# amoretti86/phylo

Measured on AMD Instinct MI355X. Metric: particle-site-likelihoods/sec, higher is better.
Workload: dtype f64; 1 GPU; primate.p N=12 S=898, GTR-init (jcmodel=false), K=2048 per GPU (K_total=2048), lambda=10, full sweep of 11 rank events; parallelism=particles sharded over 1 GPU(s), global resampling, sweeps_per_launch_set=16, contexts_in_flight=3, sweeps_in_flight=48, particles_in_flight=98304

## Files before the change

include/phylo_hip.h:

```cpp
#ifndef PHYLO_HIP_H
#define PHYLO_HIP_H

#include <stdint.h>

#ifdef __cplusplus
extern "C" {
#endif

typedef struct phylo_ctx phylo_ctx;

enum {
    PHYLO_OK = 0,
    PHYLO_EINVAL = -1,
    PHYLO_ENODEVICE = -2,
    PHYLO_EHIP = -3,
    PHYLO_ENOMEM = -4,
    PHYLO_ECOMM = -5,
    PHYLO_ESTATE = -6
};

enum {
    PHYLO_QUIRK_Q1_RAW_Q = 1u << 0,
    PHYLO_TWISTING = 1u << 1,
    PHYLO_TIME_KERNELS = 1u << 2,
// ... 98 lines not shown
                       phylo_stats* fwd, phylo_stats* bwd);
int phylo_vi_gradients_batch(phylo_ctx* ctx, const uint64_t* seeds, int G, uint32_t flags, int jc, const double* vars, double* logZ,
                             double* grads, phylo_stats* fwd, phylo_stats* bwd);
int phylo_vi_apply(int n_taxa, int jc, double* vars, const double* grads, int kind, double lr, double beta1, double beta2, double eps,
                   int64_t* t, double* m, double* v);

int phylo_debug_stamps(phylo_ctx* ctx, uint64_t* out, int n);

int phylo_debug_reverse_lists(int N, int K, const int64_t* ancestors, const int32_t* child, int early_free, int rows_form,
                              const int32_t* lookahead_nodes, int n_lookahead, int32_t* lists, int64_t n_lists, int32_t* meta,
                              int n_meta);

int phylo_debug_lookahead_lists(int N, int K, int S, int M, const int32_t* roots_ad, int32_t* slow_flag, int32_t* image,
                                int64_t n_image, int32_t* meta, int n_meta);

int phylo_debug_reverse_plan(int N, int K, int K_local, int S, int world, int twisted, int marks, uint32_t switches, int64_t n_slow,
                             int TS, int64_t coeff_wgs, int passes_in_flight, uint32_t* mask);
int phylo_debug_sweep_plan(int N, int K, int K_local, int S, int G, int M, int world, int transport, uint32_t flags, uint32_t switches,
                           uint32_t* mask, int32_t* launches);
int phylo_debug_sweep_chain(int N, int K, int K_local, int S, int G, int M, int world, int transport, uint32_t flags, uint32_t switches,
                            int multi_min, int scan_ancestors, int32_t* out);
int phylo_debug_sweep_chain_of(phylo_ctx* ctx, int32_t* taken);
int phylo_debug_scan_ancestors(phylo_ctx* ctx, const double* logw, int Kg, int G, const uint64_t* seeds, uint32_t r_next, int32_t* anc,
                               int32_t* list, int32_t* cnt);
int phylo_debug_scan_form(phylo_ctx* ctx, int Kg, int multi_min, int wanted);
int phylo_debug_persist_plan(int N, int K, int S, int G, uint32_t flags, uint32_t switches, int world, int transport, int n_cus,
                             int blocks_per_cu, int persist_wgs, int persist_nt, int64_t* out);
int phylo_debug_persist_of(phylo_ctx* ctx, int32_t* nt, int32_t* Wg, int32_t* m, int64_t* lds);
int phylo_debug_pack_leaf_codes(const uint8_t* codes, int N, int S, uint8_t* packed, int64_t cap, int64_t* need);
int phylo_debug_site_patterns(const uint8_t* codes, int N, int S, int32_t* U, int32_t* rep, uint16_t* image, uint32_t* rep_off,
                              uint8_t* rep_leaf, int64_t rep_leaf_cap);
int phylo_debug_site_patterns_rule(int S, int U, int coded, int ntiles, int sw);
int phylo_debug_site_patterns_of(phylo_ctx* ctx, int32_t* U, int32_t* taken);
int phylo_debug_reverse_plan_batch(int N, int K, int G, int S, uint32_t switches, int64_t n_slow, int TS, int64_t coeff_wgs,
                                   int passes_in_flight, uint32_t* mask);
int phylo_debug_tree_plan(int N, int K, int G, int world, int64_t n_clades, int64_t n_topologies, int kept_whole, int force_wide,
                          int64_t summary_temp, int64_t branches_temp, int64_t* scalars, int64_t* summary_slab, int64_t* branches_slab,
                          int32_t* sort_bits, int32_t* launches);
int phylo_debug_tree_branches_of(phylo_ctx* ctx, int32_t* wide, int32_t* cbits, int32_t* tbits);

int phylo_debug_device_lists(phylo_ctx* ctx, int32_t* lists, int64_t n_lists, int32_t* meta, int n_meta, int64_t* ancestors,
                             int32_t* child);
int phylo_debug_device_lists_of(phylo_ctx* ctx, const int64_t* ancestors, const int32_t* child, int32_t* lists, int64_t n_lists,
                                int32_t* meta, int n_meta);

int phylo_tree_summary(phylo_ctx* ctx, int64_t* n_clades, int32_t* n_topologies, int32_t* n_groups, phylo_stats* perf);
int phylo_tree_summary_fetch(phylo_ctx* ctx, uint64_t* clade_bits, uint64_t* clade_weight, int32_t* clade_group, uint64_t* topo_weight,
                             int32_t* topo_count, int32_t* topo_rep, int32_t* topo_group, int32_t* particle_topo, uint64_t* u, uint64_t* U);

int phylo_tree_branches(phylo_ctx* ctx, phylo_stats* perf);
int phylo_tree_branches_fetch(phylo_ctx* ctx, double* clade_stats, double* leaf_stats, int32_t* topo_clades, double* topo_stats);

int phylo_rell(phylo_ctx* ctx, int T, int S, const double* site_lik_TxS, int B, uint64_t seed, double* obs_T, int32_t* best_B,
               int64_t* wins_T, double* rep_loglik_TxB, int32_t* counts_BxS, double* site_loglik_TxS, phylo_stats* perf);
int phylo_debug_rell_host(int T, int S, const double* site_lik_TxS, int b0, int nB, uint64_t seed, int32_t* counts, double* x,
                          double* rl);
int phylo_rell_multiscale(phylo_ctx* ctx, int T, int S, const double* site_lik_TxS, int K, const int32_t* draws_K, int B, uint64_t seed,
                          double* obs_T, int64_t* wins_KxT, int32_t* best_KxB, double* rep_loglik_KxTxB, int32_t* counts_KxBxS,
                          phylo_stats* perf);
int phylo_debug_rell_multiscale_host(int T, int S, const double* site_lik_TxS, int K, const int32_t* draws_K, int k0, int b0, int nB,
                                     uint64_t seed, int32_t* counts, double* rl, int32_t* best);

int phylo_math_probe(phylo_ctx* ctx, int op, const double* x, const double* y, int n, double* out);

int phylo_debug_frechet(phylo_ctx* ctx, int form, const double* A_nx16, const double* E_nx16, int n, double* L_nx16);

// ... 18 lines not shown
```

phylo_amd/_ffi.py:

```python
from __future__ import annotations

import ctypes as C
import os

import numpy as np

_HERE = os.path.dirname(os.path.abspath(__file__))
LIB_PATH = os.path.join(_HERE, "csrc", "libphylo_hip.so")

PHYLO_OK = 0
QUIRK_Q1_RAW_Q = 1 << 0
TWISTING = 1 << 1
TIME_KERNELS = 1 << 2
EAGER_NODES = 1 << 3
KEEP_GRAPH = 1 << 4
ONE_LAUNCH = 1 << 5
FLAGS_DEFAULT = QUIRK_Q1_RAW_Q
COMM_ID_BYTES = 128

EXPORTS = [
    "phylo_version", "phylo_last_error", "phylo_device_count", "phylo_create", "phylo_destroy",
    "phylo_set_leaves", "phylo_set_model", "phylo_expm_batched", "phylo_cond_likelihood_K",
    "phylo_forest_loglik", "phylo_tree_loglik", "phylo_trees_loglik", "phylo_trees_loglik_rates", "phylo_trees_grad", "phylo_trees_grad_rates", "phylo_trees_grad_model", "phylo_trees_nni", "phylo_trees_nni_rates", "phylo_rell", "phylo_debug_rell_host", "phylo_rell_multiscale", "phylo_debug_rell_multiscale_host", "phylo_debug_tree_schedule", "phylo_resample", "phylo_log_zsmc", "phylo_sweep",
    "phylo_sweep_async", "phylo_sweep_batch_async", "phylo_sweep_batch_begin", "phylo_sweep_fetch_logz", "phylo_sweep_begin", "phylo_sweep_step", "phylo_sweep_step_a", "phylo_sweep_step_group", "phylo_sweep_finish", "phylo_sweep_fetch",
    "phylo_synchronize", "phylo_sweep_node", "phylo_sweep_backward", "phylo_sweep_backward_batch",
    "phylo_tree_summary", "phylo_tree_summary_fetch", "phylo_tree_branches", "phylo_tree_branches_fetch",
    "phylo_math_probe", "phylo_debug_frechet", "phylo_debug_stamps", "phylo_debug_reverse_lists", "phylo_debug_lookahead_lists", "phylo_debug_reverse_plan", "phylo_debug_reverse_plan_batch", "phylo_debug_sweep_plan", "phylo_debug_sweep_chain", "phylo_debug_sweep_chain_of", "phylo_debug_scan_ancestors", "phylo_debug_pack_leaf_codes", "phylo_debug_site_patterns", "phylo_debug_site_patterns_rule", "phylo_debug_site_patterns_of", "phylo_debug_tree_plan", "phylo_debug_tree_branches_of", "phylo_debug_scan_form", "phylo_debug_persist_plan", "phylo_debug_persist_of", "phylo_debug_device_lists", "phylo_debug_device_lists_of", "phylo_debug_remote_cache", "phylo_debug_site_product",
    "phylo_vi_gradients", "phylo_vi_gradients_batch", "phylo_vi_apply",
    "phylo_site_tile", "phylo_set_site_tile", "phylo_get_site_tile",
    "phylo_comm_unique_id", "phylo_comm_init", "phylo_comm_share", "phylo_comm_allgather", "phylo_comm_max", "phylo_comm_barrier",
    "phylo_comm_exchange_kind",
]


class PhyloError(RuntimeError):
    def __init__(self, code, msg):
        super().__init__("libphylo_hip error %d: %s" % (code, msg))
        self.code = code


class Stats(C.Structure):
    _fields_ = [("sweep_ms", C.c_double), ("merge_ms", C.c_double), ("merge_launches", C.c_int32),
                ("n_launches", C.c_int32), ("units", C.c_double), ("alg_bytes", C.c_double)]


_lib = None


def load():
    global _lib
    if _lib is None:
        if not os.path.exists(LIB_PATH):
            raise OSError("%s not found: build it with phylo_amd/csrc/build.sh (needs hipcc); "
                          "there is no CPU fallback" % LIB_PATH)
        lib = C.CDLL(LIB_PATH)
        lib.phylo_version.restype = C.c_char_p
        lib.phylo_last_error.restype = C.c_char_p
        lib.phylo_last_error.argtypes = [C.c_void_p]
        _lib = lib
    return _lib
# ... 125 lines not shown


SITE_PATTERN_SWITCH = {"0": 0, None: 1, "force": 2}


def debug_site_patterns(codes):
    lib = load()
    cd = np.ascontiguousarray(codes, dtype=np.uint8)
    if cd.ndim != 2:
        raise ValueError("codes must be [N][S]")
    N, S = cd.shape
    nC = -(-(-(-S // 64)) // 16)
    U = C.c_int32(0)
    rep = np.full(S, -1, dtype=np.int32)
    image = np.full(nC * 1024, 0xffff, dtype=np.uint16)
    rep_off = np.full(1024, 0xffffffff, dtype=np.uint32)
    rep_leaf = np.full(N * 1024, 0xff, dtype=np.uint8)
    rc = lib.phylo_debug_site_patterns(_ptr(cd), C.c_int(N), C.c_int(S), C.byref(U), _ptr(rep), _ptr(image), _ptr(rep_off), _ptr(rep_leaf),
                                       C.c_int64(rep_leaf.size))
    if rc:
        raise PhyloError(rc, lib.phylo_last_error(None).decode())
    u = U.value
    return {"U": u, "rep": rep[:u].copy(), "image": image.reshape(nC, 2, 64, 8) if u <= 8191 else None,
            "rep_off": rep_off if u <= 512 else None,
            "rep_leaf": rep_leaf[:N * 1024 * (-(-(-(-u // 64)) // 16))].reshape(N, -1, 64, 16) if u <= 512 else None}


def debug_site_patterns_rule(S, U, coded=True, ntiles=1, switch=None):
    lib = load()
    rc = lib.phylo_debug_site_patterns_rule(C.c_int(S), C.c_int(U), C.c_int(int(coded)), C.c_int(ntiles), C.c_int(SITE_PATTERN_SWITCH[switch]))
    if rc < 0:
        raise PhyloError(rc, lib.phylo_last_error(None).decode())
    return bool(rc)


TREE_SUMMARY_BUFS = ("u", "U", "bits", "kA", "kB", "val", "scan", "weight", "srt", "hp", "o_cbits", "o_cw", "o_tw", "child", "slot", "o_cg",
                     "o_tn", "o_trep", "o_tg", "o_ptopo", "vA", "vB", "flag", "sid", "cid", "seg_start", "count", "group", "first", "tid", "pos",
                     "err", "vC", "vD", "temp")
TREE_BRANCHES_BUFS = ("ebr", "lbr", "gbl", "gbr", "o_cs", "o_ls", "o_ts", "wA", "wB", "cpos", "kA", "kB", "vA", "vB", "cstart", "toff", "o_tc",
                      "temp")


def debug_tree_plan(N, K, G=1, world=1, n_clades=1, n_topologies=1, kept_whole=False, summary_temp=0, branches_temp=0, force_wide=False):
    lib = load()
    ns, nb = len(TREE_SUMMARY_BUFS), len(TREE_BRANCHES_BUFS)
    sc = (C.c_int64 * 13)()
    ss, bs = (C.c_int64 * (2 * ns + 1))(), (C.c_int64 * (2 * nb + 1))()
    bits, launches = (C.c_int32 * 17)(), (C.c_int32 * 2)()
    rc = lib.phylo_debug_tree_plan(C.c_int(N), C.c_int(K), C.c_int(G), C.c_int(world), C.c_int64(n_clades), C.c_int64(n_topologies),
                                   C.c_int(int(kept_whole)), C.c_int(int(force_wide)), C.c_int64(summary_temp), C.c_int64(branches_temp),
                                   sc, ss, bs, bits, launches)
    if rc:
        raise PhyloError(rc, lib.phylo_last_error(None).decode())
    out = dict(zip(("R", "L", "W", "E", "Emax", "Kg", "cbits", "tbits"), sc[:8]))
    out["wide"], out["gather"] = bool(sc[8]), bool(sc[9])
    if (sc[11], sc[12]) != (ns, nb):
        raise RuntimeError("TREE_SUMMARY_BUFS / TREE_BRANCHES_BUFS do not name the library's buffers")
    for key, names, a in (("summary_slab", TREE_SUMMARY_BUFS, ss), ("branches_slab", TREE_BRANCHES_BUFS, bs)):
        n = len(names)
        out[key] = {"offsets": dict(zip(names, a[:n])), "sizes": dict(zip(names, a[n:2 * n])), "total": a[2 * n]}
    out["sort_bits"] = list(bits[:sc[10]])
    out["summary_launches"], out["branches_launches"] = launches[0], launches[1]
    return out


SCAN_FORMS = ("multi", "lds512", "lds1024", "in_place")
# ... 648 lines not shown
        self._owner = owner
        world = owner.K // owner.K_local
        self.K_local = self.K // world
        self.k0 = (owner.k0 // owner.K_local) * self.K_local

    def comm_allgather_columns(self, a):
        a = np.ascontiguousarray(a)
        world = self.K // self.K_local
        if world == 1:
            return a
        out = np.empty((world,) + a.shape, dtype=a.dtype)
        self._check(self._lib.phylo_comm_allgather(self._h, _ptr(a), C.c_size_t(a.nbytes), _ptr(out)))
        return np.concatenate(list(out), axis=-1)

    def comm_allgather_blob(self, a):
        a = np.ascontiguousarray(a)
        world = self.K // self.K_local
        if world == 1:
            return a[None]
        out = np.empty((world,) + a.shape, dtype=a.dtype)
        self._check(self._lib.phylo_comm_allgather(self._h, _ptr(a), C.c_size_t(a.nbytes), _ptr(out)))
        return out

    def debug_remote_cache(self):
        used, cap = C.c_int(0), C.c_int(0)
        self._check(self._lib.phylo_debug_remote_cache(self._h, C.byref(used), C.byref(cap)))
        return used.value, cap.value

    def debug_site_patterns(self):
        U, taken = C.c_int32(0), C.c_int32(0)
        self._check(self._lib.phylo_debug_site_patterns_of(self._h, C.byref(U), C.byref(taken)))
        return U.value, bool(taken.value)

    def debug_tree_branches(self):
        wide, cbits, tbits = C.c_int32(0), C.c_int32(0), C.c_int32(0)
        self._check(self._lib.phylo_debug_tree_branches_of(self._h, C.byref(wide), C.byref(cbits), C.byref(tbits)))
        return {'wide': bool(wide.value), 'cbits': cbits.value, 'tbits': tbits.value}

    def debug_scan_form(self, Kg, wanted=True):
        rc = self._lib.phylo_debug_scan_form(self._h, C.c_int(Kg), C.c_int(0), C.c_int(int(wanted)))
        if rc < 0:
            raise PhyloError(rc, self._lib.phylo_last_error(self._h).decode())
        return SCAN_FORMS[rc]

    def debug_sweep_chain(self):
        taken = C.c_int32(0)
        self._check(self._lib.phylo_debug_sweep_chain_of(self._h, C.byref(taken)))
        return bool(taken.value)

    def debug_scan_ancestors(self, logw, seeds, r_next):
        w = np.ascontiguousarray(logw, dtype=np.float64)
        if w.ndim != 2:
            raise ValueError("logw must be [G][Kg]")
        G, Kg = w.shape
        sd = np.ascontiguousarray(seeds, dtype=np.uint64)
        if sd.shape != (G,):
            raise ValueError("one seed per group")
        anc = np.full((G, Kg), -2, dtype=np.int32)
        lst = np.full((G, Kg), -2, dtype=np.int32)
        cnt = np.full(G, -2, dtype=np.int32)
        self._check(self._lib.phylo_debug_scan_ancestors(self._h, _ptr(w), C.c_int(Kg), C.c_int(G), _ptr(sd), C.c_uint32(r_next), _ptr(anc),
                                                         _ptr(lst), _ptr(cnt)))
        return anc, lst, cnt

    def debug_persist(self):
        nt, Wg, m, lds = C.c_int32(0), C.c_int32(0), C.c_int32(0), C.c_int64(0)
# ... 29 lines not shown
```

phylo_amd/csrc/phylo_hip.hip:

```cpp
#include "../../include/phylo_hip.h"

#include <cstring>
#include <hip/hip_runtime.h>
#include <hip/hip_ext.h>
#include <rocprim/device/device_radix_sort.hpp>

#include <cstdarg>
#include <cstdio>
#include <cstdlib>
#include <atomic>
#include <chrono>
#include <mutex>
#include <string>
#include <vector>

#include "phylo_comm.h"
#include "phylo_kernels.h"
#include "phylo_packed_codes.h"
#include "phylo_site_patterns.h"
#include "phylo_persist.h"
#include "phylo_grad.h"
#include "phylo_revlists_dev.h"
#include "phylo_sweep_plan.h"
#include "phylo_train.h"
// ... 14 lines not shown
namespace {

thread_local std::string g_last_error;

struct DevBuf {
    void* p = nullptr;
    size_t bytes = 0;
};

}

struct sweep_run {
    uint64_t seed = 0;
    uint32_t flags = 0;
    int M = 1, launches = 0, next_r = 0;
    bool active = false;
    int a_done_r = -1;
    sweep_plan plan{};
    sweep_chain_form chain{};
};

struct env_switches {
    bool eager_nodes = false, rehearse_sharded = false, replicated_book = false, no_leaf_codes = false, one_launch = false,
         persist_stamps = false, grad_one_stream = false, grad_two_streams = false, rev_host_lists = false, no_remote_cache = false,
         no_p2p = false, grad_rows_chain = false, grad_coeff_chain = false, tree_wide_keys = false;
    int persist_wgs = 0;
    unsigned long long p2p_wait_ticks = PK_P2P_WAIT_TICKS;
    size_t p2p_copy_words = 65536;
    int persist_nt = 256;
    int remote_cache_cap = 0;
    int scan_multi_min = 4096;
    int scan_ancestors = 1;
    int site_patterns = PK_PAT_AUTO;
    int trees_chunk = 0;
    int rell_chunk = 0;
    void read() {
        eager_nodes = getenv("PHYLO_EAGER_NODES") != nullptr;
        rehearse_sharded = getenv("PHYLO_REHEARSE_SHARDED") != nullptr;
        replicated_book = getenv("PHYLO_REPLICATED_BOOK") != nullptr;
        grad_rows_chain = getenv("PHYLO_GRAD_ROWS_CHAIN") != nullptr;
        grad_coeff_chain = getenv("PHYLO_GRAD_COEFF_CHAIN") != nullptr;
        no_leaf_codes = getenv("PHYLO_NO_LEAF_CODES") != nullptr;
        one_launch = getenv("PHYLO_ONE_LAUNCH") != nullptr;
        persist_stamps = getenv("PHYLO_PERSIST_STAMPS") != nullptr;
        grad_one_stream = getenv("PHYLO_GRAD_ONE_STREAM") != nullptr;
        grad_two_streams = getenv("PHYLO_GRAD_TWO_STREAMS") != nullptr;
        rev_host_lists = getenv("PHYLO_REV_HOST_LISTS") != nullptr;
        no_remote_cache = getenv("PHYLO_NO_REMOTE_CACHE") != nullptr;
        { const char* e = getenv("PHYLO_TREE_WIDE_KEYS"); tree_wide_keys = e && atoi(e) != 0; }
        { const char* e = getenv("PHYLO_REMOTE_CACHE_CAP"); remote_cache_cap = e ? atoi(e) : 0; }
        { const char* e = getenv("PHYLO_SITE_PATTERNS"); site_patterns = !e ? PK_PAT_AUTO : !strcmp(e, "force") ? PK_PAT_FORCE : atoi(e) == 0 ? PK_PAT_OFF : PK_PAT_AUTO; }
        { const char* e = getenv("PHYLO_SCAN_MULTI_MIN"); scan_multi_min = e ? atoi(e) : 4096; }
        { const char* e = getenv("PHYLO_SCAN_ANCESTORS"); scan_ancestors = e ? atoi(e) : 1; }
        { const char* e = getenv("PHYLO_TREES_CHUNK"); trees_chunk = e ? atoi(e) : 0; }
        { const char* e = getenv("PHYLO_RELL_CHUNK"); rell_chunk = e ? atoi(e) : 0; }
        { const char* e = getenv("PHYLO_P2P"); no_p2p = e && atoi(e) == 0; }
        { const char* e = getenv("PHYLO_P2P_COPY_WORDS"); p2p_copy_words = e ? (size_t)atol(e) : 65536; }
        { const char* e = getenv("PHYLO_P2P_WAIT_S"); p2p_wait_ticks = e && atof(e) > 0 ? (unsigned long long)(atof(e) * 1e8) : PK_P2P_WAIT_TICKS; }
        const char* w = getenv("PHYLO_PERSIST_WGS");
        persist_wgs = w ? atoi(w) : 0;
        const char* t = getenv("PHYLO_PERSIST_NT");
        persist_nt = persist_nt_of(t ? atoi(t) : 0);
    }
};

struct phylo_ctx {
    int device = 0;
    env_switches env;
    int n_cus = 0;
    unsigned long long* d_rdraw = nullptr;
    unsigned long long* d_pctr = nullptr;
    unsigned long long pctr_base = 0;
    int pctr_Wg = 0, pctr_G = 0;
    bool pctr_dirty = false;
    int persist_blocks_per_cu = -1;
    bool last_persistent = false;
    int last_pp_nt = 0, last_pp_Wg = 0, last_pp_m = 0;
    size_t last_pp_lds = 0;
    unsigned long long* d_stamps = nullptr;
    int K = 0, N = 0, S = 0, A = 4;
    int Kloc = 0, k0 = 0;
    int rank = 0, world = 1;
    uint32_t flags = 0;
    hipStream_t stream = nullptr;
    hipEvent_t ev0 = nullptr, ev1 = nullptr;
    std::vector<hipEvent_t> kev;
    std::string err;
    bool have_leaves = false, have_model = false, swept = false, state_ready = false;
    int jc = 0;
    std::vector<double> h_lam_l, h_lam_r, h_ldf;
    double *d_Q = nullptr, *d_pi = nullptr, *d_lam_l = nullptr, *d_lam_r = nullptr, *d_ldf = nullptr;
    double* d_leaves = nullptr;
    uint8_t* d_leaf_codes = nullptr;
    uint8_t* d_leaf_packed = nullptr;
    uint8_t* d_pat = nullptr;
    int pat_U = 0;
    bool leaves_coded = false;
    uint32_t* d_pair_hist = nullptr;
    bool hist_ready = false, codes_valid = false;
    double* d_pool = nullptr;
    double* d_nodell = nullptr;
    double *d_bl = nullptr, *d_br = nullptr, *d_Pmat = nullptr;
    double *d_logw = nullptr, *d_ll = nullptr;
    double* d_aux = nullptr;
    unsigned long long* d_rec = nullptr;
    int tile_override = 0;
    int site_tile = 0, ntiles = 1;
    double* d_tilev = nullptr;
    double* d_lse = nullptr;
    uint64_t* d_group_seeds = nullptr;
    char* d_tables = nullptr;
    int32_t *d_roots[2] = {nullptr, nullptr}, *d_cnt[2] = {nullptr, nullptr};
    double* d_rootll[2] = {nullptr, nullptr};
    const char** d_tab_ptrs = nullptr;
    int32_t* d_child = nullptr;
    unsigned int* d_mark = nullptr;
    double* d_sync = nullptr;
    bool p2p = false;
    char* d_xslab = nullptr;
    size_t xslab_bytes = 0, x_flag_off[2] = {0, 0};
    char** d_xslab_ptrs = nullptr;
    unsigned long long x_epoch[2] = {0, 0};
    bool last_lazy = false;
    bool leaves_newer = false;
    int32_t* d_merges = nullptr;
    int64_t* d_anc = nullptr;
    uint64_t* d_cdf[2] = {nullptr, nullptr};
    int32_t* d_anc_next = nullptr;
    int32_t* d_adopt_list = nullptr;
    int32_t* d_adopt_cnt = nullptr;
// ... 201 lines not shown
    c->d_ad_off = c->d_ad_idx = c->d_par_off = c->d_par_idx = nullptr;
    c->d_heavy = c->d_chunk_beg = c->d_chunk_cnt = nullptr;
    c->d_slow_flag = c->d_slow_idx = c->d_adp = nullptr;
    if (c->h_csr_p) (void)hipHostFree(c->h_csr_p);
    if (c->h_anc_p) (void)hipHostFree(c->h_anc_p);
    if (c->h_child_p) (void)hipHostFree(c->h_child_p);
    if (c->h_rad_p) (void)hipHostFree(c->h_rad_p);
    if (c->h_pub) (void)hipHostFree(c->h_pub);
    if (c->d_row_done) (void)hipFree(c->d_row_done);
    c->d_row_done = nullptr;
    if (c->h_dlmeta) (void)hipHostFree(c->h_dlmeta);
    c->h_dlmeta = c->hd_dlmeta = nullptr;
    if (c->ev_dl) (void)hipEventDestroy(c->ev_dl);
    c->ev_dl = nullptr;
    if (c->dl_graph) (void)hipGraphExecDestroy(c->dl_graph);
    c->dl_graph = nullptr;
    c->h_pub = c->hd_pub = nullptr;
    c->h_csr_p = c->h_child_p = c->h_rad_p = nullptr;
    c->h_anc_p = nullptr;
    if (c->ev_gcopy) (void)hipEventDestroy(c->ev_gcopy);
    c->ev_gcopy = nullptr;
    c->graph_ready = false;
    c->last_graph = false;
    if (c->d_stamps) (void)hipFree(c->d_stamps);
    c->d_stamps = nullptr;
    if (c->d_rdraw) (void)hipFree(c->d_rdraw);
    if (c->d_pctr) (void)hipFree(c->d_pctr);
    c->d_rdraw = c->d_pctr = nullptr;
    c->pctr_base = 0;
    c->pctr_Wg = c->pctr_G = 0;
    c->pctr_dirty = false;
    if (c->d_tilev) (void)hipFree(c->d_tilev);
    c->d_tilev = nullptr;
    void* ptrs[] = {c->d_pool, c->d_nodell, c->d_bl, c->d_br, c->d_Pmat, c->d_logw, c->d_ll, c->d_aux, c->d_lse, c->d_group_seeds,
                    c->d_tables, (void*)c->d_tab_ptrs, c->d_child, c->d_merges, c->d_anc,
                    c->d_cdf[0], c->d_cdf[1], c->d_anc_next, c->d_adopt_list, c->d_adopt_cnt, c->d_counter, (void*)c->d_pool_ptrs, c->d_mark, c->d_sync, c->d_mirror, c->d_cache, c->d_rec};
    for (void* p : ptrs)
        if (p) (void)hipFree(p);
    c->d_pool = c->d_nodell = c->d_bl = c->d_br = c->d_Pmat = c->d_logw = c->d_ll = c->d_aux = c->d_lse = nullptr;
    c->d_group_seeds = nullptr;
    c->d_rec = nullptr;
    c->d_roots[0] = c->d_roots[1] = c->d_cnt[0] = c->d_cnt[1] = c->d_child = c->d_merges = nullptr;
    c->d_anc = nullptr;
    c->d_cdf[0] = c->d_cdf[1] = nullptr;
    c->d_anc_next = c->d_adopt_list = c->d_adopt_cnt = nullptr;
    c->d_counter = nullptr;
    c->d_rootll[0] = c->d_rootll[1] = nullptr;
    c->d_tables = nullptr;
    c->d_tab_ptrs = nullptr;
    c->d_pool_ptrs = nullptr;
    c->d_mark = nullptr;
    c->d_sync = nullptr;
    c->d_mirror = nullptr;
    c->d_cache = nullptr;
    c->cache_cap = 0;
}

int alloc_sweep_state(phylo_ctx* c) {
    free_sweep_state(c);
    c->state_ready = false;
    const size_t R = (size_t)c->N - 1, K = c->K, Kl = c->Kloc, N = c->N, S = c->S;
    CHK(dalloc(c, &c->d_pool, R * Kl * S * 4));
    c->p2p = c->comm.transport != 0 && c->world > 1 && !c->env.no_p2p && R >= 2;
    if (c->p2p) {
        const size_t al = 32;
        auto up = [&](size_t n) { return (n + al - 1) / al * al; };
// ... 317 lines not shown
        }
        if (hipStreamCreateWithFlags(&c->stream, hipStreamNonBlocking) != hipSuccess) { rc = fail(c, PHYLO_EHIP, "hipStreamCreate failed"); break; }
        if (hipEventCreate(&c->ev0) != hipSuccess || hipEventCreate(&c->ev1) != hipSuccess) { rc = fail(c, PHYLO_EHIP, "hipEventCreate failed"); break; }
        if ((rc = dalloc(c, &c->d_Q, 20 + 2 * (size_t)N)) != PHYLO_OK) break;
        c->d_pi = c->d_Q + 16;
        c->d_lam_l = c->d_Q + 20;
        c->d_lam_r = c->d_Q + 20 + N;
        if ((rc = dalloc(c, &c->d_ldf, (size_t)N + 1)) != PHYLO_OK) break;
        if ((rc = dalloc(c, &c->d_leaves, (size_t)N * S * 4)) != PHYLO_OK) break;
        if ((rc = dalloc(c, &c->d_leaf_codes, pk_leaf_image_bytes(N, S))) != PHYLO_OK) break;
        c->d_leaf_packed = c->d_leaf_codes + pk_packed_offset(N, S);
        c->d_pat = c->d_leaf_codes + pk_pat_offset(N, S);
        c->h_ldf.resize((size_t)N + 1);
        for (int cnt = 0; cnt <= N; ++cnt) c->h_ldf[cnt] = host_log_double_factorial(2 * (cnt > 2 ? cnt : 2) - 3);
        if (hipMemcpy(c->d_ldf, c->h_ldf.data(), ((size_t)N + 1) * 8, hipMemcpyHostToDevice) != hipSuccess) { rc = fail(c, PHYLO_EHIP, "ldf upload failed"); break; }
    } while (0);
    if (rc != PHYLO_OK) {
        g_last_error = c->err;
        phylo_destroy(c);
        return rc;
    }
    *out = c;
    return PHYLO_OK;
}

int phylo_destroy(phylo_ctx* c) {
    if (!c) return PHYLO_OK;
    (void)hipSetDevice(c->device);
    if (c->stream) (void)hipStreamSynchronize(c->stream);
    if (c->gstream) (void)hipStreamSynchronize(c->gstream);
    if (c->bgstream) (void)hipStreamSynchronize(c->bgstream);
    phylo_comm_destroy(&c->comm);
    free_sweep_state(c);
    void* ptrs[] = {c->d_Q, c->d_ldf, c->d_leaves, c->d_leaf_codes};
    for (void* p : ptrs)
        if (p) (void)hipFree(p);
    for (auto& b : c->scratch)
        if (b.p) (void)hipFree(b.p);
    for (hipEvent_t e : c->kev) (void)hipEventDestroy(e);
    if (c->ev0) (void)hipEventDestroy(c->ev0);
    if (c->ev1) (void)hipEventDestroy(c->ev1);
    if (c->evb0) (void)hipEventDestroy(c->evb0);
    if (c->evb1) (void)hipEventDestroy(c->evb1);
    if (c->ev_model) (void)hipEventDestroy(c->ev_model);
    if (c->ev_tb0) (void)hipEventDestroy(c->ev_tb0);
    if (c->ev_tb1) (void)hipEventDestroy(c->ev_tb1);
    if (c->ev_tl0) (void)hipEventDestroy(c->ev_tl0);
    if (c->ev_tl1) (void)hipEventDestroy(c->ev_tl1);
    if (c->ev_rl0) (void)hipEventDestroy(c->ev_rl0);
    if (c->ev_rl1) (void)hipEventDestroy(c->ev_rl1);
    if (c->ev_rm0) (void)hipEventDestroy(c->ev_rm0);
    if (c->ev_rm1) (void)hipEventDestroy(c->ev_rm1);
    if (c->ev_tg0) (void)hipEventDestroy(c->ev_tg0);
    if (c->ev_tg1) (void)hipEventDestroy(c->ev_tg1);
    if (c->ev_tr0) (void)hipEventDestroy(c->ev_tr0);
    if (c->ev_tr1) (void)hipEventDestroy(c->ev_tr1);
    if (c->ev_tn0) (void)hipEventDestroy(c->ev_tn0);
    if (c->ev_tn1) (void)hipEventDestroy(c->ev_tn1);
    if (c->ev_tm0) (void)hipEventDestroy(c->ev_tm0);
    if (c->ev_tm1) (void)hipEventDestroy(c->ev_tm1);
    if (c->ev_tq0) (void)hipEventDestroy(c->ev_tq0);
    if (c->ev_tq1) (void)hipEventDestroy(c->ev_tq1);
    if (c->ev_ts0) (void)hipEventDestroy(c->ev_ts0);
    if (c->ev_ts1) (void)hipEventDestroy(c->ev_ts1);
    if (c->ev_gfork) (void)hipEventDestroy(c->ev_gfork);
    if (c->ev_gjoin) (void)hipEventDestroy(c->ev_gjoin);
    if (c->ev_gup) (void)hipEventDestroy(c->ev_gup);
    if (c->ev_bgfork) (void)hipEventDestroy(c->ev_bgfork);
    if (c->ev_bgdone) (void)hipEventDestroy(c->ev_bgdone);
    if (c->bgstream) (void)hipStreamDestroy(c->bgstream);
    for (hipEvent_t e : c->ev_coeff)
        if (e) (void)hipEventDestroy(e);
    if (c->gstream) (void)hipStreamDestroy(c->gstream);
    if (c->h_model_p) (void)hipHostFree(c->h_model_p);
    if (c->ev_leaves) (void)hipEventDestroy(c->ev_leaves);
    if (c->h_leaves_p) (void)hipHostFree(c->h_leaves_p);
    if (c->stream) (void)hipStreamDestroy(c->stream);
    delete c;
    return PHYLO_OK;
}

int phylo_site_tile(int S) { return pm_site_tile(S); }

int phylo_get_site_tile(const phylo_ctx* c) { return c ? c->site_tile : 0; }

int phylo_set_site_tile(phylo_ctx* c, int T) {
    CHK(bind(c));
    if (T < 0 || (T & 63) || T > PK_MAX_SITE_TILE)
        return fail(c, PHYLO_EINVAL, "the site tile must be a multiple of 64 in [64, %d], or 0 for the default (got %d)", PK_MAX_SITE_TILE, T);
    if (c->comm.transport != 0) return fail(c, PHYLO_ESTATE, "phylo_set_site_tile must precede phylo_comm_init (peers map the sweep state)");
    HIPCHK(c, hipStreamSynchronize(c->stream));
    c->tile_override = T;
    c->site_tile = T ? T : pm_site_tile(c->S);
    c->ntiles = (c->S + c->site_tile - 1) / c->site_tile;
    free_sweep_state(c);
    c->state_ready = false;
    c->swept = false; ++c->sweep_serial;
    c->ts_done = c->tb_done = false;
    return PHYLO_OK;
}

int phylo_set_leaves(phylo_ctx* c, const double* genome) {
    CHK(bind(c));
    if (!genome) return fail(c, PHYLO_EINVAL, "genome_NxSxA is NULL");
    const size_t rows = (size_t)c->N * c->S;
    const size_t code_bytes = pk_leaf_image_bytes(c->N, c->S);
    const bool pinned = rows * 32 + code_bytes <= ((size_t)8 << 20);
    std::vector<uint8_t> codes_v;
    uint8_t* codes = nullptr;
    if (pinned) {
        if (!c->h_leaves_p) {
            HIPCHK(c, hipHostMalloc((void**)&c->h_leaves_p, rows * 32 + code_bytes));
            HIPCHK(c, hipEventCreateWithFlags(&c->ev_leaves, hipEventDisableTiming));
        } else {
            HIPCHK(c, hipEventSynchronize(c->ev_leaves));
        }
        memcpy(c->h_leaves_p, genome, rows * 32);
        HIPCHK(c, hipMemcpyAsync(c->d_leaves, c->h_leaves_p, rows * 32, hipMemcpyHostToDevice, c->stream));
        codes = (uint8_t*)c->h_leaves_p + rows * 32;
    } else {
        HIPCHK(c, hipMemcpyAsync(c->d_leaves, genome, rows * 32, hipMemcpyHostToDevice, c->stream));
        codes_v.resize(code_bytes);
        codes = codes_v.data();
    }
    {
        bool ok = true;
        for (size_t i = 0; i < rows && ok; ++i) {
            const double* x = genome + i * 4;
            int ones = 0, zeros = 0, last = 0;
            for (int j = 0; j < 4; ++j) {
                if (pm_bits(x[j]) == pm_bits(1.0)) { ++ones; last = j; }
                else if (pm_bits(x[j]) == 0) ++zeros;
            }
            if (ones == 1 && zeros == 3) codes[i] = (uint8_t)last;
            else if (ones == 4) codes[i] = 4;
            else ok = false;
        }
        c->codes_valid = ok;
        c->leaves_coded = ok && !c->env.no_leaf_codes;
        c->hist_ready = false;
        c->pat_U = 0;
        if (ok) {
            pk_pack_leaf_codes(codes, c->N, c->S, codes + pk_packed_offset(c->N, c->S));
            c->pat_U = pk_pat_build(codes, c->N, c->S, codes + pk_pat_offset(c->N, c->S));
            const size_t up_bytes = c->pat_U <= PK_PAT_MAX_U ? code_bytes : pk_codes_image_bytes(c->N, c->S);
            HIPCHK(c, hipMemcpyAsync(c->d_leaf_codes, codes, up_bytes, hipMemcpyHostToDevice, c->stream));
        }
    }
    if (pinned) HIPCHK(c, hipEventRecord(c->ev_leaves, c->stream));
    c->have_leaves = true;
    c->last_graph = c->last_graph_twist = false;
    c->leaves_newer = true;
    CHK(refresh_leaf_ll(c));
    if (!pinned) HIPCHK(c, hipStreamSynchronize(c->stream));
    return PHYLO_OK;
}

int phylo_set_model(phylo_ctx* c, const double* Q16, const double* pi4, const double* lam_l, const double* lam_r,
                    int jc69_closed_form) {
    CHK(bind(c));
    if (!Q16 || !pi4 || !lam_l || !lam_r) return fail(c, PHYLO_EINVAL, "NULL model pointer");
    const int R = c->N - 1;
    for (int i = 0; i < R; ++i)
        if (!(lam_l[i] > 0.0) || !(lam_r[i] > 0.0)) return fail(c, PHYLO_EINVAL, "branch rates must be positive");
    c->h_lam_l.assign(lam_l, lam_l + R);
    c->h_lam_r.assign(lam_r, lam_r + R);
    c->jc = jc69_closed_form ? 1 : 0;
    const size_t npack = 20 + 2 * (size_t)c->N;
    if (!c->h_model_p) {
        HIPCHK(c, hipHostMalloc((void**)&c->h_model_p, npack * 8));
        HIPCHK(c, hipEventCreateWithFlags(&c->ev_model, hipEventDisableTiming));
    } else {
        HIPCHK(c, hipEventSynchronize(c->ev_model));
    }
    double* pack = c->h_model_p;
    memset(pack, 0, npack * 8);
    memcpy(pack, Q16, 16 * 8);
    memcpy(pack + 16, pi4, 4 * 8);
    memcpy(pack + 20, lam_l, (size_t)R * 8);
// ... 1179 lines not shown
        CHK(launch_check(c, "ptnr_finish"));
        launches += 3;
        HIPCHK(c, hipEventRecord(c->ev_tm1, c->stream));
        HIPCHK(c, hipMemcpyAsync(loglik_T + t0, d_out, (size_t)n * 8, hipMemcpyDeviceToHost, c->stream));
        HIPCHK(c, hipMemcpyAsync(delta + (size_t)t0 * 2 * R, d_dout, (size_t)n * 2 * R * 8, hipMemcpyDeviceToHost, c->stream));
        HIPCHK(c, hipStreamSynchronize(c->stream));
        float ms = 0.f;
        HIPCHK(c, hipEventElapsedTime(&ms, c->ev_tm0, c->ev_tm1));
        ms_total += ms;
    }
    if (perf) {
        phylo_stats st{};
        st.sweep_ms = ms_total;
        st.n_launches = launches;
        st.units = (double)T * S * R * C;
        st.alg_bytes = 96.0 * st.units;
        *perf = st;
    }
    return PHYLO_OK;
}

static void sweep_facts_flags(sweep_facts& f, uint32_t flags) {
    f.twisting = (flags & PHYLO_TWISTING) != 0; f.keep_graph = (flags & PHYLO_KEEP_GRAPH) != 0;
    f.eager_nodes = (flags & PHYLO_EAGER_NODES) != 0; f.time_kernels = (flags & PHYLO_TIME_KERNELS) != 0;
}

static sweep_facts sweep_facts_of(const phylo_ctx* c, uint32_t flags, int M, int G) {
    sweep_facts f{};
    f.N = c->N; f.K = c->K; f.Kloc = c->Kloc; f.S = c->S; f.G = G; f.M = M; f.world = c->world; f.ntiles = c->ntiles;
    f.transport = c->comm.transport != 0; f.device_exchange = c->p2p; f.jc = c->jc != 0; f.coded_leaves = c->codes_valid;
    sweep_facts_flags(f, flags);
    f.env_eager_nodes = c->env.eager_nodes; f.env_rehearse_sharded = c->env.rehearse_sharded;
    f.env_replicated_book = c->env.replicated_book;
    return f;
}

static int sweep_bind(phylo_ctx* c) {
    CHK(bind(c));
    c->run.active = false;
    return PHYLO_OK;
}
static int sweep_ready(phylo_ctx* c) {
    if (!c->have_leaves || !c->have_model)
        return fail(c, PHYLO_ESTATE, "phylo_set_leaves and phylo_set_model must be called before a sweep");
    if (!c->state_ready) {
        CHK(ensure_sweep_state(c));
        CHK(refresh_leaf_ll(c));
    }
    return PHYLO_OK;
}

static void sweep_publish(phylo_ctx* c, bool lazy, bool graph, int G, bool final_missing, int merge_events, int launches, double units) {
    c->swept = true;
    c->leaves_newer = false;
    c->last_lazy = lazy;
    c->last_graph = graph;
    c->last_G = G;
    c->last_final_missing = final_missing;
    c->n_merge_events = merge_events;
    c->stats.n_launches = launches;
    c->stats.units = units;
    c->stats.alg_bytes = 96.0 * units;
}

static int sweep_alloc_twist(phylo_ctx* c, int M) {
    const int N = c->N, K = c->K, Kl = c->Kloc;
// ... 42 lines not shown
        c->htw_rows = 0;
        CHK(dalloc(c, &c->d_htw_b, rows * 2));
        CHK(dalloc(c, &c->d_htw_P, rows * 32));
        CHK(dalloc(c, &c->d_hpot, rows));
        CHK(dalloc(c, &c->d_tau, rows));
        CHK(dalloc(c, &c->d_twpart, rows * PG_PART));
        c->htw_rows = rows;
    }
    if (!c->d_hroots_ad) {
        CHK(dalloc(c, &c->d_hroots_ad, (size_t)R * K * N));
        CHK(dalloc(c, &c->d_hchosen, (size_t)R * K));
        CHK(dalloc(c, &c->d_ctw, (size_t)R * K * N));
        CHK(dalloc(c, &c->d_twnode, (size_t)R * K * PG_NODEG));
        CHK(dalloc(c, &c->d_joff, (size_t)R + 1));
        HIPCHK(c, hipHostMalloc((void**)&c->h_rad_p, (size_t)R * K * N * 4));
        HIPCHK(c, hipHostGetDevicePointer((void**)&c->hd_rad, c->h_rad_p, 0));
    }
    HIPCHK(c, hipMemcpyAsync(c->d_joff, c->h_joff.data(), ((size_t)R + 1) * 8, hipMemcpyHostToDevice, c->stream));
    return PHYLO_OK;
}

static int sweep_alloc(phylo_ctx* c, const sweep_plan& p, int M) {
    if (p.twist) CHK(sweep_alloc_twist(c, M));
    while (p.timek && (int)c->kev.size() < 2 * p.R) {
        hipEvent_t e;
        HIPCHK(c, hipEventCreate(&e));
        c->kev.push_back(e);
    }
    if (p.graph) {
        CHK(ensure_graph_state(c));
        if (p.twist) CHK(sweep_alloc_twist_history(c, M));
    }
    if (p.want_rdraw && !c->d_rdraw) CHK(dalloc(c, &c->d_rdraw, (size_t)p.R * c->K));
    return PHYLO_OK;
}

static int sweep_prologue(phylo_ctx* c, const sweep_plan& p, uint64_t seed, const uint64_t* group_seeds) {
    const int N = c->N, K = c->K, Kl = c->Kloc, R = p.R, G = p.G;
    const size_t mark_words = ((size_t)R * K + R + 3) & ~(size_t)3;
    int32_t* t_roots = p.graph ? c->d_hroots : c->d_roots[0];
    int32_t* t_cnt = p.graph ? c->d_hcnt : c->d_cnt[0];
    double* t_rootll = p.graph ? c->d_hrootll : c->d_rootll[0];
    if (!p.twist) {
        if (G > 1) HIPCHK(c, hipMemcpyAsync(c->d_group_seeds, group_seeds, (size_t)G * 8, hipMemcpyHostToDevice, c->stream));
        pk_prologue_args pa{};
        pa.Q = c->d_Q; pa.lam_l = c->d_lam_l; pa.lam_r = c->d_lam_r; pa.jc = c->jc; pa.seed = seed; pa.R = R; pa.Kloc = Kl; pa.k0 = c->k0;
        pa.bl = c->d_bl; pa.br = c->d_br; pa.Pmat = c->d_Pmat; pa.Kg = p.Kg;
        pa.group_seeds = G > 1 ? (const uint64_t*)c->d_group_seeds : (const uint64_t*)nullptr;
        pa.rdraw = p.want_rdraw ? c->d_rdraw : (unsigned long long*)nullptr;
        pa.roots = t_roots; pa.cnt = t_cnt; pa.rootll = t_rootll; pa.nodell = c->d_nodell; pa.K = K; pa.N = N;
        pa.mark = p.lazy ? c->d_mark : (unsigned int*)nullptr;
        pa.mark_words = p.lazy ? (unsigned int)mark_words : 0u;
        const int NT = p.sorted_prologue ? 256 : 64;
        pa.draw_blocks = p.sorted_prologue ? cdiv(2L * R * Kl, PK_DRAW_ITEMS) : cdiv(2L * R * Kl, 64);
        pa.init_blocks = cdiv((long)K * N, 4 * NT);
        pa.mark_blocks = p.lazy ? cdiv((long)mark_words, 4 * NT) : 0;
        const int rdraw_blocks = p.want_rdraw ? cdiv((long)(R - 1) * K, NT) : 0;
        const dim3 pgrid(pa.draw_blocks + pa.init_blocks + pa.mark_blocks + rdraw_blocks);
        if (p.sorted_prologue) hipLaunchKernelGGL(pk_sweep_prologue_sorted, pgrid, dim3(256), 0, c->stream, pa);
        else hipLaunchKernelGGL(pk_sweep_prologue, pgrid, dim3(64), 0, c->stream, pa);
        CHK(launch_check(c, "pk_sweep_prologue"));
    } else {
        if (p.lazy) HIPCHK(c, hipMemsetAsync(c->d_mark, 0, mark_words * sizeof(unsigned int), c->stream));
        hipLaunchKernelGGL(pk_init_tables, dim3(cdiv((long)K * N, 256)), dim3(256), 0, c->stream, t_roots, t_cnt, t_rootll,
                           (const double*)c->d_nodell, K, N);
    }
    CHK(launch_check(c, "pk_init_tables"));
    if (c->d_mirror) HIPCHK(c, hipMemsetAsync(c->d_mirror, 0, ((size_t)R * K + 4) * 4, c->stream));
    return PHYLO_OK;
}

static int sweep_begin_impl(phylo_ctx* c, uint64_t seed, uint32_t flags, int M, const uint64_t* group_seeds, int G) {
    CHK(sweep_bind(c));
    const sweep_facts f = sweep_facts_of(c, flags, M, G);
    char why[160];
    if (sweep_refuses_batch(f, k_sweep_limits, why, sizeof why)) return fail(c, PHYLO_EINVAL, "%s", why);
    CHK(sweep_ready(c));
    if (sweep_refuses_form(f, k_sweep_limits, why, sizeof why)) return fail(c, PHYLO_EINVAL, "%s", why);
    const sweep_plan p = sweep_plan_form(f, k_sweep_limits);
    CHK(sweep_alloc(c, p, M));
    c->swept = false; ++c->sweep_serial;
    HIPCHK(c, hipEventRecord(c->ev0, c->stream));
    CHK(sweep_prologue(c, p, seed, group_seeds));
// ... 134 lines not shown
    a.timeout_word = c->d_counter + 1;
    a.wait_ticks = c->env.p2p_wait_ticks;
    const size_t words = (size_t)n_arrays * count * (size_t)(c->world - 1);
    if (words > c->env.p2p_copy_words) {
        const size_t wgs = (words + 4095) / 4096;
        hipLaunchKernelGGL(pk_p2p_copy, dim3((unsigned)(wgs < 512 ? wgs : 512)), dim3(1024), 0, c->stream, a);
        CHK(launch_check(c, "pk_p2p_copy"));
        a.n_seg = 0;
    }
    hipLaunchKernelGGL(pk_p2p_exchange, dim3(1), dim3(1024), 0, c->stream, a);
    return launch_check(c, "pk_p2p_exchange");
}

static bool pat_on(const phylo_ctx* c) { return pk_pat_take(c->S, c->pat_U, c->leaves_coded, c->ntiles, c->env.site_patterns); }

static pk_rank_args rank_args(const phylo_ctx* c, int r) {
    const sweep_plan& p = c->run.plan;
    const int N = c->N, K = c->K, Kl = c->Kloc, cur = r & 1, nxt = cur ^ 1;
    const size_t plane = (size_t)K * N;
    pk_rank_args b{};
    b.r = r; b.n = N - r; b.N = N; b.S = c->S; b.K = K; b.Kloc = Kl; b.k0 = c->k0;
    b.seed = c->run.seed; b.flags = c->run.flags;
    b.Kg = p.Kg; b.group_seeds = p.G > 1 ? c->d_group_seeds : nullptr;
    b.no_store = (r == p.R - 1 && p.no_store_last) ? 1 : 0;
    if (p.graph) {
        b.roots_old = c->d_hroots + plane * r; b.cnt_old = c->d_hcnt + plane * r;
        b.roots_new = c->d_hroots + plane * (r + 1); b.cnt_new = c->d_hcnt + plane * (r + 1);
        b.rootll_old = c->d_hrootll + plane * r; b.rootll_new = c->d_hrootll + plane * (r + 1);
        b.pos_hist = c->d_pos + plane * r;
    } else {
        b.roots_old = c->d_roots[cur]; b.cnt_old = c->d_cnt[cur];
        b.roots_new = c->d_roots[nxt]; b.cnt_new = c->d_cnt[nxt];
        b.rootll_old = c->d_rootll[cur]; b.rootll_new = c->d_rootll[nxt];
    }
    if (p.local_book) {
        b.tab_ptrs = c->d_tab_ptrs;
        b.tab_off_rootll = (size_t)cur * K * N * 8;
        b.tab_off_roots = (size_t)16 * K * N + (size_t)cur * K * N * 4;
        b.tab_off_cnt = (size_t)24 * K * N + (size_t)cur * K * N * 4;
    }
    b.cdf = c->d_cdf[cur];
    b.rdraw = p.want_rdraw ? c->d_rdraw + (size_t)r * K : nullptr;
    b.ll_prev = r > 0 ? c->d_ll + (size_t)(r - 1) * K : nullptr;
    b.nodell = c->d_nodell;
    b.ldf = c->d_ldf; b.ldf_n = N;
    b.bl = c->d_bl; b.br = c->d_br;
    b.lam_l = c->h_lam_l[r]; b.lam_r = c->h_lam_r[r];
    b.loglam_l = pm_log(b.lam_l); b.loglam_r = pm_log(b.lam_r);
    b.ll_tilde0 = pm_log(1.0 / (double)p.Kg);
    b.leaves = c->d_leaves; b.pool = c->d_pool; b.pool_ptrs = c->d_pool_ptrs;
    b.mirror = (p.twist || p.replicated_book) ? nullptr : c->d_mirror; b.cache = c->d_cache; b.cache_cap = c->cache_cap;
    b.leaf_codes = c->leaves_coded ? c->d_leaf_codes : nullptr;
    b.leaf_packed = c->leaves_coded ? c->d_leaf_packed : nullptr;
    b.packed_leaf_bytes = pk_packed_leaf_bytes(c->S);
    b.Pmat = c->d_Pmat + (size_t)r * Kl * 32;
    b.pi = c->d_pi;
    b.logw_r = c->d_logw + (size_t)r * K;
    b.ll_r = c->d_ll + (size_t)r * K;
    b.merges = c->d_merges; b.ancestors = c->d_anc;
    b.child = c->d_child + (size_t)r * Kl * 2; b.aux = c->d_aux;
    b.rec = p.use_rec ? c->d_rec : nullptr;
    b.lazy = p.lazy ? 1 : 0; b.mark = c->d_mark; b.child_all = c->d_child; b.Pmat_all = c->d_Pmat;
    b.T = c->site_tile; b.ntiles = c->ntiles; b.tilev = c->d_tilev;
    if (c->run.chain.taken && r > 0) {
        b.anc_in = c->d_anc_next; b.adopt_list = c->d_adopt_list; b.adopt_cnt = c->d_adopt_cnt;
        b.item_waves = c->run.chain.item_waves; b.item_parts = c->run.chain.parts;
// ... 51 lines not shown
    ta.codes = p.twist_ll ? c->d_leaf_codes : nullptr;
    ta.bl_r = c->d_bl + (size_t)r * Kl; ta.br_r = c->d_br + (size_t)r * Kl;
    ta.own_tables = p.twist_tables ? 0 : 1;
    ta.wbuf = c->d_twbuf;
    hipLaunchKernelGGL(pk_twist_adopt_draws, dim3(K + cdiv(2L * Kl * ta.J, 64)), dim3(64), 0, c->stream, ta, (const double*)c->d_Q, c->jc);
    CHK(launch_check(c, "pk_twist_adopt_draws"));
    if (p.twist_ll) {
        hipLaunchKernelGGL(pk_twist_potentials_ll, dim3((ta.J + 7) / 8, Kl), dim3(256), 0, c->stream, ta);
        CHK(launch_check(c, "pk_twist_potentials_ll"));
    }
    const bool any_rows = !(p.twist_ll && r == 0);
    const dim3 pgrid((unsigned)((((size_t)Kl * ta.J + 7) / 8) * 8));
    if (p.timek) {
        if (any_rows) hipExtLaunchKernelGGL(pk_twist_potentials, pgrid, dim3(64), 0, c->stream, c->kev[2 * r], c->kev[2 * r + 1], 0, ta);
        else { HIPCHK(c, hipEventRecord(c->kev[2 * r], c->stream)); HIPCHK(c, hipEventRecord(c->kev[2 * r + 1], c->stream)); }
    } else if (any_rows) {
        hipLaunchKernelGGL(pk_twist_potentials, pgrid, dim3(64), 0, c->stream, ta);
    }
    CHK(launch_check(c, "pk_twist_potentials"));
    hipLaunchKernelGGL(pk_twist_choose, dim3(Kl), dim3(64), (size_t)(ta.J <= PK_TWIST_LDS_J ? ta.J : 0) * 8, c->stream, ta);
    CHK(launch_check(c, "pk_twist_choose"));
    if (p.twist_tables) {
        double* rows[1] = {c->d_chosen};
        CHK(comm_exchange(c, rows, 1, (size_t)Kl, 1));
        hipLaunchKernelGGL(pk_twist_tables, dim3(cdiv(K, 128)), dim3(128), 0, c->stream, ta);
        CHK(launch_check(c, "pk_twist_tables"));
    }
    return PHYLO_OK;
}

static int step_book(phylo_ctx* c, const pk_rank_args& b) {
    const sweep_plan& p = c->run.plan;
    const int K = c->K, w = p.book_width;
    const size_t lds = pk_book_lds_bytes(c->N);
    if (p.book_mat && b.r > 0) {
        const int lp = w < 16 ? 16 : w, per = PK_COLS / lp;
        const int bb = cdiv(K, per);
        const dim3 grid(bb + K);
        switch (lp) {
        case 16: hipLaunchKernelGGL(pk_rank_book_mat<16>, grid, dim3(PK_COLS), lds * per, c->stream, b, bb); break;
        case 32: hipLaunchKernelGGL(pk_rank_book_mat<32>, grid, dim3(PK_COLS), lds * per, c->stream, b, bb); break;
        case 64: hipLaunchKernelGGL(pk_rank_book_mat<64>, grid, dim3(PK_COLS), lds * per, c->stream, b, bb); break;
        default: return fail(c, PHYLO_ESTATE, "step_book: no pk_rank_book_mat of %d lanes", lp);
        }
        return launch_check(c, "pk_rank_book_mat");
    }
    const int per = 64 / (w > 0 ? w : 64);
    const sweep_chain_form& ch = c->run.chain;
    if (ch.taken) {
        const int items = b.r > 0 ? p.G * ch.item_waves : 0;
        const dim3 grid(items + cdiv(K, per));
        switch (w) {
        case 8: hipLaunchKernelGGL(pk_rank_book_chain<8>, grid, dim3(64), lds * per, c->stream, b, items); break;
        case 16: hipLaunchKernelGGL(pk_rank_book_chain<16>, grid, dim3(64), lds * per, c->stream, b, items); break;
        case 32: hipLaunchKernelGGL(pk_rank_book_chain<32>, grid, dim3(64), lds * per, c->stream, b, items); break;
        case 64: hipLaunchKernelGGL(pk_rank_book_chain<64>, grid, dim3(64), lds * per, c->stream, b, items); break;
        default: return fail(c, PHYLO_ESTATE, "step_book: no pk_rank_book_chain of %d lanes", w);
        }
        return launch_check(c, "pk_rank_book_chain");
    }
    const dim3 grid(cdiv(p.local_book ? c->Kloc : K, per));
    switch (w) {
    case 8: hipLaunchKernelGGL(pk_rank_book_packed<8>, grid, dim3(64), lds * per, c->stream, b); break;
    case 16: hipLaunchKernelGGL(pk_rank_book_packed<16>, grid, dim3(64), lds * per, c->stream, b); break;
    case 32: hipLaunchKernelGGL(pk_rank_book_packed<32>, grid, dim3(64), lds * per, c->stream, b); break;
    case 64: hipLaunchKernelGGL(pk_rank_book_packed<64>, grid, dim3(64), lds * per, c->stream, b); break;
    default: return fail(c, PHYLO_ESTATE, "step_book: no pk_rank_book_packed of %d lanes", w);
    }
    return launch_check(c, "pk_rank_book_packed");
}

static int step_merge(phylo_ctx* c, const pk_rank_args& b) {
    const sweep_plan& p = c->run.plan;
    const int S = c->S;
    const dim3 mgrid((unsigned)((size_t)c->Kloc * c->ntiles));
    hipEvent_t e0 = nullptr, e1 = nullptr;
    if (p.timek && !p.twist) { e0 = c->kev[2 * b.r]; e1 = c->kev[2 * b.r + 1]; }
    if (!(b.lazy || b.no_store)) {
        const size_t lds = (size_t)(c->site_tile < S ? c->site_tile : S) * 8 + 16 + PK_STORE_STAGE_BYTES;
        launch_stamped(pk_rank_merge, mgrid, dim3(PK_COLS), lds, c->stream, e0, e1, b);
    } else if (b.rec) {
        pk_pi4 pi4;
        memcpy(pi4.v, c->h_model_p + 16, sizeof pi4.v);
        pk_pat_args pat = {nullptr, nullptr, 0, 0};
        size_t lds = 0;
        if (pat_on(c)) {
            pat.pimg = (const char*)c->d_pat;
            pat.roff = (const char*)c->d_pat + pk_pat_image_bytes(S);
            pat.rep_delta = (long long)((c->d_pat + pk_pat_image_bytes(S) + pk_pat_rep_bytes()) - c->d_leaf_packed);
            pat.U = c->pat_U;
            lds = pk_pat_lds_bytes(c->pat_U);
        }
        launch_stamped(pk_rank_merge_nostore, mgrid, dim3(64), lds, c->stream, e0, e1, (const unsigned long long*)b.rec, b.Pmat, S, b.T,
                       b.ntiles, b.tilev, pi4, pat);
    } else {
        launch_stamped(pk_rank_merge_nostore_ids, mgrid, dim3(64), 0, c->stream, e0, e1, b);
    }
    return launch_check(c, "pk_rank_merge");
}

static int step_tiles(phylo_ctx* c, const pk_rank_args& b) {
    hipLaunchKernelGGL(pk_tile_epilogue, dim3(cdiv(c->Kloc, 256)), dim3(256), 0, c->stream, b);
    return launch_check(c, "pk_tile_epilogue");
}

static int step_exchange(phylo_ctx* c, int r) {
    const size_t K = c->K;
    double* rows[3] = {c->d_logw + r * K, c->d_ll + r * K, c->d_nodell + c->N + r * K};
    return comm_exchange(c, rows, 3, (size_t)c->Kloc, 0);
}

static int step_fix_rootll(phylo_ctx* c, int r) {
    const int N = c->N, K = c->K;
    double* rootll_new = c->run.plan.graph ? c->d_hrootll + (size_t)K * N * (r + 1) : c->d_rootll[(r & 1) ^ 1];
    hipLaunchKernelGGL(pk_fix_rootll, dim3(cdiv(K, 256)), dim3(256), 0, c->stream, rootll_new,
                       (const double*)(c->d_nodell + N + (size_t)r * K), K, N, N - r, c->k0, c->Kloc);
    return launch_check(c, "pk_fix_rootll");
}

// ... 1032 lines not shown
    for (int r = 0; r <= R; ++r) {
        meta[4 + r] = x.ev_chunk0[r];
        meta[4 + (R + 1) + r] = x.ev_node0[r];
    }
    return PHYLO_OK;
}

int phylo_debug_reverse_plan(int N, int K, int K_local, int S, int world, int twisted, int marks, uint32_t switches, int64_t n_slow, int TS,
                             int64_t coeff_wgs, int passes_in_flight, uint32_t* mask) {
    if (N < 2 || K < 1 || K_local < 1 || S < 1 || world < 1 || TS < 1 || n_slow < 0 || coeff_wgs < 0 || !mask)
        return fail(nullptr, PHYLO_EINVAL, "phylo_debug_reverse_plan: bad arguments");
    pg_plan_in in{};
    in.N = N; in.K = K; in.K_local = K_local; in.S = S; in.world = world;
    in.twist = twisted != 0; in.marks = marks != 0;
    in.rev_host_lists = switches & 1; in.one_stream = switches & 2; in.two_streams = switches & 4;
    in.rows_chain = switches & 8; in.coeff_chain = switches & 16;
    in.dl_max_k = PG_DL_MAX_K;
    pg_plan p = pg_plan_form(in);
    pg_plan_chains(p, (long)n_slow, TS, (long)coeff_wgs, passes_in_flight, N - 1);
    *mask = pg_plan_mask(p);
    return PHYLO_OK;
}

int phylo_debug_sweep_plan(int N, int K, int K_local, int S, int G, int M, int world, int transport, uint32_t flags, uint32_t switches,
                           uint32_t* mask, int32_t* launches) {
    if (N < 2 || N > PK_MAX_TAXA || K < 1 || K_local < 1 || K_local > K || S < 1 || world < 1 || !mask || !launches)
        return fail(nullptr, PHYLO_EINVAL, "phylo_debug_sweep_plan: bad arguments");
    sweep_facts f{};
    f.N = N; f.K = K; f.Kloc = K_local; f.S = S; f.G = G; f.M = M; f.world = world;
    f.ntiles = (S + pm_site_tile(S) - 1) / pm_site_tile(S);
    f.transport = transport != 0;
    sweep_facts_flags(f, flags);
    f.env_eager_nodes = switches & 1; f.env_rehearse_sharded = switches & 2; f.env_replicated_book = switches & 4;
    f.jc = switches & 8; f.coded_leaves = switches & 16; f.device_exchange = switches & 32;
    char why[160];
    if (sweep_refuses_batch(f, k_sweep_limits, why, sizeof why) || sweep_refuses_form(f, k_sweep_limits, why, sizeof why))
        return fail(nullptr, PHYLO_EINVAL, "%s", why);
    const sweep_plan p = sweep_plan_form(f, k_sweep_limits);
    *mask = sweep_plan_mask(p);
    for (int r = -1; r <= p.R; ++r) launches[r + 1] = sweep_plan_launches(p, r);
    return PHYLO_OK;
}

int phylo_debug_sweep_chain(int N, int K, int K_local, int S, int G, int M, int world, int transport, uint32_t flags, uint32_t switches,
                            int multi_min, int scan_ancestors, int32_t* out) {
    if (N < 2 || N > PK_MAX_TAXA || K < 1 || K_local < 1 || K_local > K || S < 1 || world < 1 || !out)
        return fail(nullptr, PHYLO_EINVAL, "phylo_debug_sweep_chain: bad arguments");
    sweep_facts f{};
    f.N = N; f.K = K; f.Kloc = K_local; f.S = S; f.G = G; f.M = M; f.world = world;
    f.ntiles = (S + pm_site_tile(S) - 1) / pm_site_tile(S);
    f.transport = transport != 0;
    sweep_facts_flags(f, flags);
    f.env_eager_nodes = switches & 1; f.env_rehearse_sharded = switches & 2; f.env_replicated_book = switches & 4;
    f.jc = switches & 8; f.coded_leaves = switches & 16; f.device_exchange = switches & 32;
    char why[160];
    if (sweep_refuses_batch(f, k_sweep_limits, why, sizeof why) || sweep_refuses_form(f, k_sweep_limits, why, sizeof why))
        return fail(nullptr, PHYLO_EINVAL, "%s", why);
    const sweep_chain_form ch = sweep_chain_form_of(sweep_plan_form(f, k_sweep_limits), S, multi_min, scan_ancestors, k_sweep_limits);
    out[0] = ch.taken ? 1 : 0; out[1] = ch.item_waves; out[2] = ch.parts;
    return PHYLO_OK;
}

int phylo_debug_sweep_chain_of(phylo_ctx* c, int32_t* taken) {
    if (!c || !taken) return fail(c, PHYLO_EINVAL, "phylo_debug_sweep_chain_of: NULL argument");
    *taken = c->last_chain;
    return PHYLO_OK;
}
// ... 32 lines not shown
    return PHYLO_OK;
}

int phylo_debug_site_patterns(const uint8_t* codes, int N, int S, int32_t* U, int32_t* rep, uint16_t* image, uint32_t* rep_off,
                              uint8_t* rep_leaf, int64_t rep_leaf_cap) {
    if (N < 1 || S < 1 || !codes || !U) return fail(nullptr, PHYLO_EINVAL, "phylo_debug_site_patterns: bad arguments");
    std::vector<int32_t> pat((size_t)S), rp((size_t)S);
    *U = pk_pat_columns(codes, N, S, pat.data(), rp.data());
    if (rep) memcpy(rep, rp.data(), (size_t)*U * sizeof(int32_t));
    if (image && *U <= PK_PAT_IMAGE_MAX_U) pk_pat_pack_image(pat.data(), S, *U, image);
    if (rep_off && *U <= PK_PAT_MAX_U) pk_pat_rep_offsets(rp.data(), *U, rep_off);
    if (rep_leaf && *U <= PK_PAT_MAX_U) {
        if (rep_leaf_cap < (int64_t)pk_packed_bytes(N, *U))
            return fail(nullptr, PHYLO_EINVAL, "phylo_debug_site_patterns: the representative leaf image takes %lld bytes (got %lld)",
                        (long long)pk_packed_bytes(N, *U), (long long)rep_leaf_cap);
        pk_pat_rep_leaf_image(codes, N, S, rp.data(), *U, rep_leaf, pk_packed_leaf_bytes(*U));
    }
    return PHYLO_OK;
}

int phylo_debug_site_patterns_rule(int S, int U, int coded, int ntiles, int sw) {
    if (S < 1 || U < 0 || ntiles < 1 || sw < PK_PAT_OFF || sw > PK_PAT_FORCE) {
        (void)fail(nullptr, PHYLO_EINVAL, "phylo_debug_site_patterns_rule: bad arguments");
        return -1;
    }
    return pk_pat_take(S, U, coded != 0, ntiles, sw) ? 1 : 0;
}

int phylo_debug_site_patterns_of(phylo_ctx* c, int32_t* U, int32_t* taken) {
    if (!c || !U || !taken) return fail(c, PHYLO_EINVAL, "phylo_debug_site_patterns_of: NULL argument");
    if (!c->have_leaves) return fail(c, PHYLO_ESTATE, "phylo_debug_site_patterns_of needs leaves");
    *U = c->pat_U;
    *taken = pat_on(c) ? 1 : 0;
    return PHYLO_OK;
}

int phylo_debug_tree_plan(int N, int K, int G, int world, int64_t n_clades, int64_t n_topologies, int kept_whole, int force_wide,
                          int64_t summary_temp, int64_t branches_temp, int64_t* scalars, int64_t* summary_slab, int64_t* branches_slab,
                          int32_t* sort_bits, int32_t* launches) {
    if (K < 1 || G < 1 || K % G != 0 || N > PK_MAX_TAXA || world < 1 || summary_temp < 0 || branches_temp < 0 || !scalars || !summary_slab ||
        !branches_slab || !sort_bits || !launches)
        return fail(nullptr, PHYLO_EINVAL, "phylo_debug_tree_plan: bad arguments");
    char why[160];
    const pt_facts f{N, K, G, world};
    if (pt_refuses(f, why, sizeof why)) return fail(nullptr, PHYLO_EINVAL, "%s", why);
    const pb_facts fb{N, K, G, world, n_clades, n_topologies, kept_whole != 0, force_wide != 0};
    if (pb_refuses(fb, why, sizeof why)) return fail(nullptr, PHYLO_ESTATE, "%s", why);
    pt_plan p = pt_plan_form(f);
    pt_plan_slab(p, (size_t)summary_temp);
    pb_plan q = pb_plan_form(fb);
    pb_plan_slab(q, (size_t)branches_temp);
    unsigned bits[PT_MAX_WORDS + 9];
    const int n_sorts = pt_plan_sorts(p, bits);
    for (int i = 0; i < n_sorts; ++i) sort_bits[i] = (int32_t)bits[i];
    const int64_t sc[] = {p.R, p.L, p.W, p.E, p.Emax, p.Kg, q.cbits, q.tbits, q.wide, q.gather, n_sorts, pt_slab::NBUF, pb_slab::NBUF};
    memcpy(scalars, sc, sizeof sc);
    for (int i = 0; i < pt_slab::NBUF; ++i) { summary_slab[i] = (int64_t)p.slab.off[i]; summary_slab[pt_slab::NBUF + i] = (int64_t)p.slab.bytes[i]; }
    summary_slab[2 * pt_slab::NBUF] = (int64_t)p.slab.total;
    for (int i = 0; i < pb_slab::NBUF; ++i) { branches_slab[i] = (int64_t)q.slab.off[i]; branches_slab[pb_slab::NBUF + i] = (int64_t)q.slab.bytes[i]; }
    branches_slab[2 * pb_slab::NBUF] = (int64_t)q.slab.total;
    launches[0] = pt_plan_launches(p);
    launches[1] = pb_plan_launches(q);
    return PHYLO_OK;
}

int phylo_debug_scan_form(phylo_ctx* c, int Kg, int multi_min, int wanted) {
// ... 662 lines not shown
```

phylo_amd/csrc/phylo_kernels.h:

```cpp
#pragma once
#include <hip/hip_runtime.h>
#include <stdint.h>

#include "phylo_math.h"
#include "phylo_packed_codes.h"
#include "phylo_site_patterns.h"

#define PK_COLS 256
#define PK_AUX 8
#define PK_MAX_TAXA 512
#define PK_MAX_GROUPS 64

enum { AUX_SUM_REM = 0, AUX_FPRIOR, AUX_LPRIOR, AUX_RPRIOR, AUX_LL_TILDE, AUX_PAREN, AUX_LOGV, AUX_Q };
#define PK_REC 16
enum { REC_BASE_L = PK_AUX, REC_BASE_R, REC_NODELL, REC_ROOTLL, REC_LL, REC_LOGW, REC_FLAGS  };
#define PK_REC_SLOTS (REC_FLAGS + 1)
static_assert(PK_REC_SLOTS <= PK_REC && PK_REC_SLOTS <= 16, "one lane per slot: with 16 lanes or more per particle the bookkeeping writes the record in one trip (pk_book_tail)");

__device__ __forceinline__ double pk_block_canon_sum(double col, double* sh4) {
#pragma unroll
    for (int off = 1; off < 64; off <<= 1) col = col + __shfl_xor(col, off, 64);
    __syncthreads();
    if ((threadIdx.x & 63) == 0) sh4[threadIdx.x >> 6] = col;
    __syncthreads();
// ... 106 lines not shown

__device__ __forceinline__ void pk_sweep_draws_body(int t, const double* __restrict__ Q, const double* __restrict__ lam_l,
                                                    const double* __restrict__ lam_r, int jc, uint64_t seed, int R, int K,
                                                    int k0, double* __restrict__ bl, double* __restrict__ br,
                                                    double* __restrict__ Pmat, int Kg, const uint64_t* __restrict__ group_seeds) {
    if (t >= 2 * R * K) return;
    const int side = t & 1, i = t >> 1;
    const int r = i / K, k = i - r * K;
    int kp = k0 + k;
    if (group_seeds) { const int g = kp / Kg; seed = group_seeds[g]; kp -= g * Kg; }
    const pm_u32x4 x = pm_philox4x32((uint32_t)kp, (uint32_t)r, PM_STREAM_BRANCH, 0u, seed);
    const double b = side ? (-pm_log(pm_unit_oc(x.z, x.w))) / lam_r[r] : (-pm_log(pm_unit_oc(x.x, x.y))) / lam_l[r];
    (side ? br : bl)[i] = b;
    double q[16], p[16];
#pragma unroll
    for (int j = 0; j < 16; ++j) q[j] = Q[j];
    if (jc) pm_jc69(b, p); else pm_expm4(q, b, p);
    double* out = Pmat + (size_t)i * 32 + side * 16;
#pragma unroll
    for (int j = 0; j < 16; ++j) out[j] = p[j];
}

struct pk_prologue_args {
    const double *Q, *lam_l, *lam_r;
    int jc, R, Kloc, k0, Kg;
    uint64_t seed;
    double *bl, *br, *Pmat;
    const uint64_t* group_seeds;
    unsigned long long* rdraw;
    int32_t *roots, *cnt;
    double* rootll;
    const double* nodell;
    int K, N;
    unsigned int* mark;
    unsigned int mark_words;
    int draw_blocks, init_blocks, mark_blocks;
};
#define PK_DRAW_ITEMS 1024
__device__ __forceinline__ void pk_sweep_draws_sorted(int wg, const pk_prologue_args& p) {
    __shared__ double sb[PK_DRAW_ITEMS];
    __shared__ unsigned short slist[PK_DRAW_ITEMS];
    __shared__ int scount[8];
    const int tid = threadIdx.x, NT = 256;
    const int total = 2 * p.R * p.Kloc, base = wg * PK_DRAW_ITEMS;
    if (tid < 8) scount[tid] = 0;
    double q[16];
#pragma unroll
    for (int j = 0; j < 16; ++j) q[j] = p.Q[j];
    double qn = 0.0;
#pragma unroll
    for (int j = 0; j < 4; ++j) {
        double cs = 0.0;
#pragma unroll
        for (int i = 0; i < 4; ++i) cs = cs + (q[i * 4 + j] < 0.0 ? -q[i * 4 + j] : q[i * 4 + j]);
        qn = cs > qn ? cs : qn;
    }
    __syncthreads();
    int cls[PK_DRAW_ITEMS / 512][2], pos[PK_DRAW_ITEMS / 512][2];
#pragma unroll
    for (int u = 0; u < PK_DRAW_ITEMS / 512; ++u) {
        const int pair = u * NT + tid, t0 = base + 2 * pair;
        cls[u][0] = cls[u][1] = -1;
        if (t0 < total) {
            const int i = t0 >> 1, r = i / p.Kloc, k = i - r * p.Kloc;
            int kp = p.k0 + k;
            uint64_t seed = p.seed;
// ... 28 lines not shown
                const int c = cls[u][sd];
                const int o = c == 0 ? off[0] : c == 1 ? off[1] : c == 2 ? off[2] : c == 3 ? off[3] : off[4];
                slist[o + pos[u][sd]] = (unsigned short)(2 * (u * NT + tid) + sd);
            }
    __syncthreads();
    const int nitems = total - base < PK_DRAW_ITEMS ? total - base : PK_DRAW_ITEMS;
    #pragma unroll 1
    for (int sidx = tid; sidx < nitems; sidx += NT) {
        const int li = slist[sidx], t = base + li;
        double pm[16];
        pm_expm4(q, sb[li], pm);
        double* out = p.Pmat + (size_t)(t >> 1) * 32 + (t & 1) * 16;
#pragma unroll
        for (int j = 0; j < 16; ++j) out[j] = pm[j];
    }
}

template <int NT, bool SORTED>
__device__ __forceinline__ void pk_sweep_prologue_body(const pk_prologue_args& p) {
    const int b = blockIdx.x;
    if (b < p.draw_blocks) {
        if constexpr (SORTED) pk_sweep_draws_sorted(b, p);
        else pk_sweep_draws_body(b * NT + (int)threadIdx.x, p.Q, p.lam_l, p.lam_r, p.jc, p.seed, p.R, p.Kloc, p.k0, p.bl, p.br, p.Pmat, p.Kg,
                                 p.group_seeds);
    } else if (b < p.draw_blocks + p.init_blocks) {
        const int i0 = ((b - p.draw_blocks) * NT + (int)threadIdx.x) * 4;
#pragma unroll
        for (int u = 0; u < 4; ++u) {
            const int i = i0 + u;
            if (i < p.K * p.N) {
                p.roots[i] = i % p.N;
                p.cnt[i] = 1;
                p.rootll[i] = p.nodell[i % p.N];
            }
        }
    } else if (b < p.draw_blocks + p.init_blocks + p.mark_blocks) {
        const unsigned int w = (unsigned int)((b - p.draw_blocks - p.init_blocks) * NT + (int)threadIdx.x) * 4u;
        if (w < p.mark_words) *reinterpret_cast<uint4*>(p.mark + w) = make_uint4(0u, 0u, 0u, 0u);
    } else {
        const long i = (long)(b - p.draw_blocks - p.init_blocks - p.mark_blocks) * NT + (int)threadIdx.x + p.K;
        if (i < (long)p.R * p.K) {
            const int r = (int)(i / p.K);
            int kp = (int)(i - (long)r * p.K);
            uint64_t seed = p.seed;
            if (p.group_seeds) { const int g = kp / p.Kg; seed = p.group_seeds[g]; kp -= g * p.Kg; }
            const pm_u32x4 d = pm_philox4x32((uint32_t)kp, (uint32_t)r, PM_STREAM_RESAMPLE, 0u, seed);
            p.rdraw[i] = ((unsigned long long)d.y << 32) | d.x;
        }
    }
}
__global__ __launch_bounds__(64) void pk_sweep_prologue(const pk_prologue_args p) { pk_sweep_prologue_body<64, false>(p); }
__global__ __launch_bounds__(256) void pk_sweep_prologue_sorted(const pk_prologue_args p) { pk_sweep_prologue_body<256, true>(p); }

__global__ __launch_bounds__(64) void pk_row_loglik(const double* __restrict__ x, const double* __restrict__ pi4,
                                                     int S, int T, double* __restrict__ out) {
    const double* row = x + (size_t)blockIdx.x * S * 4;
    double pi[4] = {pi4[0], pi4[1], pi4[2], pi4[3]};
    double tot = 0.0;
    for (int s0 = 0; s0 < S; s0 += T) {
        const int s1 = s0 + T < S ? s0 + T : S;
        pm_lp col = pm_lp_init();
        for (int s = s0 + threadIdx.x; s < s1; s += 64) {
            double v[4];
            pk_load4(row + (size_t)s * 4, v);
            pm_lp_mul(col, pk_site_lik(pi, v));
        }
// ... 261 lines not shown
    const uint8_t* leaf_codes;
    const uint8_t* leaf_packed;
    size_t packed_leaf_bytes;
    double* pool;
    const double* const* pool_ptrs;
    int32_t* mirror;
    double* cache;
    int cache_cap;
    const double* Pmat;
    const double* pi;
    double* logw_r; double* ll_r;
    int32_t* merges;
    int64_t* ancestors;
    int lazy;
    unsigned int* mark;
    const int32_t* child_all;
    const double* Pmat_all;
    int32_t* child;
    double* aux;
    int32_t* pos_hist;
    const char* const* tab_ptrs;
    size_t tab_off_rootll, tab_off_roots, tab_off_cnt;
    int Kg;
    const uint64_t* group_seeds;
    int no_store;
    const unsigned long long* rdraw;
    int T, ntiles;
    double* tilev;
    unsigned long long* rec;
    const int32_t* anc_in;
    const int32_t* adopt_list;
    const int32_t* adopt_cnt;
    int item_waves, item_parts;
};

struct pk_book_lds {
    double *ord_ll, *ord_ldf, *hbl, *hbr, *anc_ll, *ldf;
    uint32_t* key; int32_t *ro, *co, *ord_cnt;
    double* aux; int32_t* misc;
};
__host__ __device__ inline size_t pk_book_lds_bytes(int N) {
    const size_t n4 = ((size_t)N + 3) & ~(size_t)3;
    return (6 * n4 + 4) * 8 + PK_AUX * 8 + (4 * n4) * 4 + 16 ;
}
__device__ __forceinline__ pk_book_lds pk_book_carve(char* base, int N) {
    const size_t n4 = ((size_t)N + 3) & ~(size_t)3;
    pk_book_lds L;
    L.ord_ll = (double*)base;
    L.ord_ldf = L.ord_ll + n4;
    L.hbl = L.ord_ldf + n4;
    L.hbr = L.hbl + n4;
    L.anc_ll = L.hbr + n4;
    L.ldf = L.anc_ll + n4;
    L.aux = L.ldf + n4 + 4;
    L.key = (uint32_t*)(L.aux + PK_AUX);
    L.ro = (int32_t*)(L.key + n4);
    L.co = L.ro + n4;
    L.ord_cnt = L.co + n4;
    L.misc = L.ord_cnt + n4;
    return L;
}

__device__ __forceinline__ void pk_rec_write(const pk_rank_args& a, int k, int kg, int t, const pk_book_lds& L) {
    const size_t node_sz = (size_t)a.S * 4;
    unsigned long long v;
    if (t < PK_AUX) {
        v = (unsigned long long)__double_as_longlong(L.aux[t]);
    } else if (t <= REC_BASE_R) {
        const int id = L.misc[t - REC_BASE_L];
        if (id >= a.N) v = (unsigned long long)(a.pool + (size_t)(id - a.N) * node_sz);
        else if (a.leaf_codes) v = (unsigned long long)(a.leaf_packed + (size_t)id * a.packed_leaf_bytes);
        else v = (unsigned long long)(a.leaves + (size_t)id * node_sz);
    } else if (t == REC_NODELL) {
        v = (unsigned long long)(a.nodell + (a.N + a.r * a.K + kg));
    } else if (t == REC_ROOTLL) {
        v = (unsigned long long)(a.rootll_new + ((size_t)kg * a.N + (a.n - 2)));
    } else if (t == REC_LL) {
        v = (unsigned long long)(a.ll_r + kg);
    } else if (t == REC_LOGW) {
        v = (unsigned long long)(a.logw_r + kg);
    } else {
        v = a.leaf_codes ? (unsigned long long)((L.misc[0] < a.N ? 1 : 0) | (L.misc[1] < a.N ? 2 : 0)) : 0ull;
    }
    a.rec[(size_t)k * PK_REC + t] = v;
}


template <int LP>
__device__ __forceinline__ int pk_cdf_search_group(const uint64_t* cdf, int K, uint64_t R, int sl, int lane) {
    const int gshift = lane & ~(LP - 1);
    const unsigned long long gmask = LP == 64 ? ~0ull : ((1ull << (LP & 63)) - 1ull);
    int lo = 0, hi = K;
    int step = (K + LP - 1) / LP;
    int p = (sl + 1) * step - 1;
    if (p > K - 1) p = K - 1;
    const uint64_t total = cdf[K - 1];
    uint64_t c = cdf[p];
    const uint64_t thr = pm_mulhi64(R, total);
    bool done = false;
    for (;;) {
        const unsigned long long ball = __ballot(!done && c > thr);
        if (!done) {
            const unsigned long long mask = (ball >> gshift) & gmask;
            const int f = mask ? __ffsll((long long)mask) - 1 : LP - 1;
            int pf = lo + (f + 1) * step - 1;
            if (pf > hi - 1) pf = hi - 1;
            lo = lo + f * step;
            hi = pf + 1;
            if (lo >= hi) lo = hi - 1;
            if (hi - lo <= 1) done = true;
            else {
                step = (hi - lo + LP - 1) / LP;
                p = lo + (sl + 1) * step - 1;
                if (p > hi - 1) p = hi - 1;
                c = cdf[p];
            }
        }
        if (__all(done)) break;
    }
    return lo;
}

template <int LP, bool KEY_LOOP, bool ANC_IN = false>
__device__ __forceinline__ void pk_book_packed(const pk_rank_args& a, int kg, bool local, const pk_book_lds& L, int sl, int lane) {
    const int n = a.n, N = a.N, k = kg - a.k0;
    const int grp = a.group_seeds ? kg / a.Kg : 0;
    const int gbase = grp * a.Kg;
    const uint64_t seed = a.group_seeds ? a.group_seeds[grp] : a.seed;
    const uint32_t kin = (uint32_t)(kg - gbase);
    {
        #pragma unroll 1
        for (int j = sl; j <= a.r; j += LP) {
            L.hbl[j] = local ? a.bl[(size_t)j * a.Kloc + k] : 0.0;
            L.hbr[j] = local ? a.br[(size_t)j * a.Kloc + k] : 0.0;
        }
        #pragma unroll 1
        for (int j = sl; j <= a.ldf_n; j += LP) L.ldf[j] = a.ldf[j];
        const int nb = (n + 3) / 4;
        uint64_t Rdraw;
        if (ANC_IN) Rdraw = 0;
        if (KEY_LOOP && nb > LP - 1) {
            #pragma unroll 1
            for (int b = sl; b < nb; b += LP) {
                const pm_u32x4 x = pm_philox4x32(kin, (uint32_t)a.r, PM_STREAM_PAIR, (uint32_t)b, seed);
                L.key[b * 4 + 0] = x.x; L.key[b * 4 + 1] = x.y; L.key[b * 4 + 2] = x.z; L.key[b * 4 + 3] = x.w;
            }
            if (!ANC_IN) {
                const pm_u32x4 x = pm_philox4x32(kin, (uint32_t)a.r, PM_STREAM_RESAMPLE, 0u, seed);
                Rdraw = ((uint64_t)x.y << 32) | x.x;
            }
        } else {
            const bool res = !ANC_IN && sl == LP - 1;
            const pm_u32x4 x = pm_philox4x32(kin, (uint32_t)a.r, res ? PM_STREAM_RESAMPLE : PM_STREAM_PAIR, res ? 0u : (uint32_t)sl, seed);
            if (sl < nb) { L.key[sl * 4 + 0] = x.x; L.key[sl * 4 + 1] = x.y; L.key[sl * 4 + 2] = x.z; L.key[sl * 4 + 3] = x.w; }
            if (!ANC_IN) {
                const int src = (lane & ~(LP - 1)) + LP - 1;
                Rdraw = ((uint64_t)(uint32_t)__shfl((int)x.y, src, 64) << 32) | (uint32_t)__shfl((int)x.x, src, 64);
            }
        }
        int anc = kg;
        if (ANC_IN) { if (a.r > 0) anc = gbase + a.anc_in[kg]; }
        else if (a.r > 0) anc = gbase + pk_cdf_search_group<LP>(a.cdf + gbase, a.group_seeds ? a.Kg : a.K, Rdraw, sl, lane);
        const int32_t* ro = a.roots_old + (size_t)anc * N;
        const int32_t* co = a.cnt_old + (size_t)anc * N;
        const double* rl = a.rootll_old + (size_t)anc * N;
        if (a.tab_ptrs) {
            const char* base = a.tab_ptrs[anc / a.Kloc];
            ro = reinterpret_cast<const int32_t*>(base + a.tab_off_roots) + (size_t)anc * N;
            co = reinterpret_cast<const int32_t*>(base + a.tab_off_cnt) + (size_t)anc * N;
            rl = reinterpret_cast<const double*>(base + a.tab_off_rootll) + (size_t)anc * N;
        }
        #pragma unroll 1
        for (int i = sl; i < n; i += LP) { L.ro[i] = ro[i]; L.co[i] = co[i]; L.anc_ll[i] = rl[i]; }
        if (sl == 0) {
            L.misc[3] = anc;
            if (local) L.aux[AUX_LL_TILDE] = (a.r > 0) ? a.ll_prev[anc] : a.ll_tilde0;
        }
    }
    __syncthreads();
    {
        unsigned long long best = 0ull;
        #pragma unroll 1
        for (int i = sl; i < n; i += LP) {
            const unsigned long long c = ((unsigned long long)L.key[i] << 32) | (0xffffffffu - (uint32_t)i);
            best = c > best ? c : best;
        }
#pragma unroll
        for (int off = 1; off < LP; off <<= 1) {
            const unsigned long long o = __shfl_xor(best, off, 64);
            best = o > best ? o : best;
        }
        const int il = (int)(0xffffffffu - (uint32_t)best);
        best = 0ull;
        #pragma unroll 1
        for (int i = sl; i < n; i += LP) {
            const unsigned long long c = ((unsigned long long)L.key[i] << 32) | (0xffffffffu - (uint32_t)i);
            if (i != il) best = c > best ? c : best;
        }
#pragma unroll
        for (int off = 1; off < LP; off <<= 1) {
            const unsigned long long o = __shfl_xor(best, off, 64);
            best = o > best ? o : best;
        }
        const int ir = (int)(0xffffffffu - (uint32_t)best);
        int32_t* rn = a.roots_new + (size_t)kg * N;
        int32_t* cn = a.cnt_new + (size_t)kg * N;
        double* rln = a.rootll_new + (size_t)kg * N;
        #pragma unroll 1
        for (int i = sl; i < n; i += LP) {
            if (i == il || i == ir) continue;
            const unsigned long long mine = ((unsigned long long)L.key[i] << 32) | (uint32_t)i;
            int rank = 0;
            #pragma unroll 1
            for (int j = 0; j < n; ++j) {
                const unsigned long long cj = ((unsigned long long)L.key[j] << 32) | (uint32_t)j;
                rank += (j != il && j != ir && cj < mine) ? 1 : 0;
            }
            const int node = L.ro[i], c = L.co[i];
            const double xll = L.anc_ll[i];
            rn[rank] = node;
            cn[rank] = c;
            rln[rank] = xll;
            if (a.pos_hist) a.pos_hist[(size_t)kg * N + i] = rank;
            L.ord_cnt[rank] = c;
            L.ord_ll[rank] = xll;
            L.ord_ldf[rank] = L.ldf[c < a.ldf_n ? c : a.ldf_n];
        }
        if (sl == 0) {
            const int cnew = L.co[il] + L.co[ir];
            rn[n - 2] = N + a.r * a.K + kg;
            cn[n - 2] = cnew;
            L.ord_cnt[n - 2] = cnew;
            L.ord_ldf[n - 2] = L.ldf[cnew < a.ldf_n ? cnew : a.ldf_n];
            L.misc[0] = L.ro[il];
            L.misc[1] = L.ro[ir];
            if (a.pos_hist) { a.pos_hist[(size_t)kg * N + il] = -1; a.pos_hist[(size_t)kg * N + ir] = -1; }
            if (local) {
                a.merges[((size_t)a.r * a.Kloc + k) * 2 + 0] = il;
                a.merges[((size_t)a.r * a.Kloc + k) * 2 + 1] = ir;
                if (a.r > 0) a.ancestors[(size_t)(a.r - 1) * a.Kloc + k] = L.misc[3] - gbase;
            }
        }
    }
    __syncthreads();
    if (local) {
        const double* src = sl == 0 ? L.ord_ll : sl == 1 ? L.ord_ldf : sl == 2 ? L.hbl : L.hbr;
        const int cnt = sl == 0 ? n - 2 : sl == 1 ? n - 1 : sl < 4 ? a.r + 1 : 0;
        const double ca = sl == 0 ? 1.0 : sl == 1 ? -1.0 : sl == 2 ? -a.lam_l : -a.lam_r;
        const double cb = sl == 2 ? a.loglam_l : sl == 3 ? a.loglam_r : 0.0;
        const int trips = n - 1 > a.r + 1 ? n - 1 : a.r + 1;
        double acc = 0.0;
        #pragma unroll 1
        for (int j = 0; j < trips; ++j)
            if (j < cnt) acc = acc + (ca * src[j] + cb);
        int vminus = 0;
        #pragma unroll 1
        for (int p = sl; p < n - 1; p += LP) {
            const int c = L.ord_cnt[p];
            vminus += c - (c == 1 ? 1 : 0);
        }
#pragma unroll
// ... 28 lines not shown
__device__ __forceinline__ int pk_cache_claim(const pk_rank_args& a, int id) {
    int x;
    const double* src;
    if (!pk_remote_node(a, id, x, src)) return -1;
    if (__hip_atomic_load(a.mirror + x, __ATOMIC_RELAXED, __HIP_MEMORY_SCOPE_AGENT) != 0) return -1;
    int expected = 0;
    if (!__hip_atomic_compare_exchange_strong(a.mirror + x, &expected, -1, __ATOMIC_RELAXED, __ATOMIC_RELAXED, __HIP_MEMORY_SCOPE_AGENT)) return -1;
    const int slot = __hip_atomic_fetch_add(a.mirror + (size_t)(a.N - 1) * a.K, 1, __ATOMIC_RELAXED, __HIP_MEMORY_SCOPE_AGENT);
    if (slot >= a.cache_cap) {
        __hip_atomic_store(a.mirror + x, -2, __ATOMIC_RELAXED, __HIP_MEMORY_SCOPE_AGENT);
        return -1;
    }
    return slot;
}
__device__ __forceinline__ void pk_cache_fill(const pk_rank_args& a, int id, int slot, int lane) {
    typedef __attribute__((ext_vector_type(4))) unsigned int cu4;
    typedef __attribute__((address_space(1))) const cu4 gsrc_t;
    typedef __attribute__((address_space(1))) cu4 gdst_t;
    int x;
    const double* srcd;
    pk_remote_node(a, id, x, srcd);
    const char* src = (const char*)srcd;
    char* dst = (char*)(a.cache + (size_t)slot * (size_t)a.S * 4);
    const size_t bytes = (size_t)a.S * 32;
    size_t o = (size_t)lane * 16;
    for (; o + 3 * 1024 < bytes; o += 4 * 1024) {
        const cu4 v0 = *(gsrc_t*)(src + o), v1 = *(gsrc_t*)(src + o + 1024), v2 = *(gsrc_t*)(src + o + 2048), v3 = *(gsrc_t*)(src + o + 3072);
        *(gdst_t*)(dst + o) = v0; *(gdst_t*)(dst + o + 1024) = v1; *(gdst_t*)(dst + o + 2048) = v2; *(gdst_t*)(dst + o + 3072) = v3;
    }
    for (; o < bytes; o += 1024) *(gdst_t*)(dst + o) = *(gsrc_t*)(src + o);
    if (lane == 0) __hip_atomic_store(a.mirror + x, slot + 1, __ATOMIC_RELAXED, __HIP_MEMORY_SCOPE_AGENT);
}

template <int LP>
__device__ __forceinline__ void pk_book_tail(const pk_rank_args& a, int kg, bool local, bool mark, bool cache, const pk_book_lds& L,
                                             int sl, int lane) {
    if (local) {
        const int k = kg - a.k0;
#pragma unroll
        for (int t = sl; t < PK_AUX + 2; t += LP) {
            if (t < PK_AUX) a.aux[(size_t)k * PK_AUX + t] = L.aux[t];
            else a.child[k * 2 + (t - PK_AUX)] = L.misc[t - PK_AUX];
        }
        if (a.rec) {
#pragma unroll
            for (int t = sl; t < PK_REC_SLOTS; t += LP) pk_rec_write(a, k, kg, t, L);
        }
    }
    if (mark && sl == 0) a.mark[(size_t)(a.r - 1) * a.K + L.misc[3]] = 1u;
    if (cache) {
#pragma unroll
        for (int c = 0; c < 2; ++c) {
            const int id = L.misc[c];
            const int slot = (local && sl == 0) ? pk_cache_claim(a, id) : -1;
            for (int g2 = 0; g2 < 64 / LP; ++g2) {
                const int s2 = __shfl(slot, g2 * LP, 64), id2 = __shfl(id, g2 * LP, 64);
                if (s2 >= 0) pk_cache_fill(a, id2, s2, lane);
            }
        }
    }
}

template <int LP>
__global__ __launch_bounds__(64, LP == 64 ? 5 : 1) void pk_rank_book_packed(const pk_rank_args a) {
    extern __shared__ __attribute__((aligned(16))) char smem[];
    const int lane = threadIdx.x, sub = lane / LP, sl = lane & (LP - 1);
    const int count = a.tab_ptrs ? a.Kloc : a.K;
    int idx = blockIdx.x * (64 / LP) + sub;
    if (idx >= count) idx = count - 1;
    const int kg = a.tab_ptrs ? a.k0 + idx : idx;
    const pk_book_lds L = pk_book_carve(smem + (size_t)sub * pk_book_lds_bytes(a.N), a.N);
    const bool local = kg >= a.k0 && kg < a.k0 + a.Kloc;
    pk_book_packed<LP, LP == 64>(a, kg, local, L, sl, lane);
    pk_book_tail<LP>(a, kg, local, a.lazy && a.r > 0, a.mirror && a.r > 0, L, sl, lane);
}

__global__ __launch_bounds__(64) void pk_all_marks(const pk_rank_args a) {
    const int lane = threadIdx.x, sub = lane >> 4, sl = lane & 15;
    int kg = blockIdx.x * 4 + sub;
    if (kg >= a.K) kg = a.K - 1;
    const int grp = a.group_seeds ? kg / a.Kg : 0;
    const int gbase = grp * a.Kg;
    const uint64_t seed = a.group_seeds ? a.group_seeds[grp] : a.seed;
    const pm_u32x4 x = pm_philox4x32((uint32_t)(kg - gbase), (uint32_t)a.r, PM_STREAM_RESAMPLE, 0u, seed);
    const uint64_t R = ((uint64_t)x.y << 32) | x.x;
    const int anc = gbase + pk_cdf_search_group<16>(a.cdf + gbase, a.group_seeds ? a.Kg : a.K, R, sl, lane);
    if (sl == 0) a.mark[(size_t)(a.r - 1) * a.K + anc] = 1u;
}

__device__ __forceinline__ const double* pk_node_ptr(const pk_rank_args& a, int id);
template <int U = 4>
__device__ __forceinline__ void pk_materialize_node(const pk_rank_args& a, int rho, int kappa, int lane, int nthreads,
                                                    int s_begin, int s_end) {
    const int k = kappa - a.k0;
    const int32_t* ch = a.child_all + ((size_t)rho * a.Kloc + k) * 2;
    const double* Lp = pk_node_ptr(a, ch[0]);
    const double* Rp = pk_node_ptr(a, ch[1]);
    const double* P = a.Pmat_all + ((size_t)rho * a.Kloc + k) * 32;
    double Pl[16], Pr[16];
#pragma unroll
    for (int j = 0; j < 16; ++j) { Pl[j] = P[j]; Pr[j] = P[16 + j]; }
    double* out = a.pool + ((size_t)rho * a.Kloc + k) * (size_t)a.S * 4;
    for (int s = s_begin + lane; s < s_end; s += U * nthreads) {
        double Lv[U][4], Rv[U][4];
#pragma unroll
        for (int u = 0; u < U; ++u) {
            const int su = s + u * nthreads < s_end ? s + u * nthreads : s;
// ... 77 lines not shown
    unsigned long long mine = 0ull;
    #pragma unroll 2
    for (int i = tid; i < Kg; i += PK_COLS) {
        const unsigned long long t = pm_mulhi64(a.rdraw[gbase + i], total);
        if (t >= lo && t < hi) {
            int l = 0, h = cnt - 1;
            while (l < h) {
                const int m = (l + h) >> 1;
                if (gcdf[m] > t) h = m; else l = m + 1;
            }
            mine |= 1ull << l;
        }
    }
#pragma unroll
    for (int off = 1; off < 64; off <<= 1) mine |= __shfl_xor(mine, off, 64);
    if ((tid & 63) == 0 && mine) {
        if ((unsigned int)mine) atomicOr(&maskw[0], (unsigned int)mine);
        if ((unsigned int)(mine >> 32)) atomicOr(&maskw[1], (unsigned int)(mine >> 32));
    }
    __syncthreads();
    unsigned long long todo = ((unsigned long long)maskw[1] << 32) | maskw[0];
    while (todo) {
        const int j = __ffsll((long long)todo) - 1;
        todo &= todo - 1;
        pk_materialize_node<1>(a, a.r - 1, k0 + j, tid, PK_COLS, 0, a.S);
        if (tid == 0) a.mark[(size_t)(a.r - 1) * a.K + k0 + j] = 1u;
    }
}
__global__ __launch_bounds__(PK_COLS) void pk_materialize_by_draws(const pk_rank_args a, int grouped) {
    if (grouped) pk_mat_by_thresholds_grouped(a, a.k0 + (int)blockIdx.x * PK_MAT_GROUP);
    else pk_mat_by_thresholds(a, a.k0 + (int)blockIdx.x);
}

template <int LP>
__global__ __launch_bounds__(PK_COLS, 5) void pk_rank_book_mat(const pk_rank_args a, int book_blocks) {
    extern __shared__ __attribute__((aligned(16))) char smem[];
    if ((int)blockIdx.x >= book_blocks) {
        pk_mat_by_thresholds(a, (int)blockIdx.x - book_blocks);
        return;
    }
    const int tid = threadIdx.x, lane = tid & 63, sub = tid / LP, sl = tid & (LP - 1);
    int idx = blockIdx.x * (PK_COLS / LP) + sub;
    if (idx >= a.K) idx = a.K - 1;
    const int kg = idx;
    const pk_book_lds L = pk_book_carve(smem + (size_t)sub * pk_book_lds_bytes(a.N), a.N);
    pk_book_packed<LP, false>(a, kg, true, L, sl, lane);
    pk_book_tail<LP>(a, kg, true, a.r > 0, false, L, sl, lane);
}

__device__ __forceinline__ const double* pk_node_ptr(const pk_rank_args& a, int id) {
    const size_t node_sz = (size_t)a.S * 4;
    if (id < a.N) return a.leaves + (size_t)id * node_sz;
    if (a.Kloc == a.K) return a.pool + (size_t)(id - a.N) * node_sz;
    const int x = id - a.N, rho = x / a.K, kap = x - rho * a.K, owner = kap / a.Kloc;
    if (a.mirror && owner * a.Kloc != a.k0) {
        const int slot = a.mirror[x];
        if (slot > 0) return a.cache + (size_t)(slot - 1) * node_sz;
    }
    return a.pool_ptrs[owner] + ((size_t)rho * a.Kloc + (kap - owner * a.Kloc)) * node_sz;
}

typedef __attribute__((address_space(4))) const int32_t pk_ci32;
#define PK_ITEM_ROWS 2
__device__ __forceinline__ void pk_mat_listed(const pk_rank_args& a, int wg, int lane) {
    typedef __attribute__((address_space(4))) const double cdbl;
    constexpr int U = PK_ITEM_ROWS;
    const int W = a.item_waves, Q = a.item_parts, rho = a.r - 1;
    const int g = __builtin_amdgcn_readfirstlane(wg / W), w = wg - g * W;
    const int n = ((pk_ci32*)a.adopt_cnt)[g] * Q;
    if (w >= n) return;
    pk_ci32* list = (pk_ci32*)(a.adopt_list + (size_t)g * a.Kg);
    const size_t node_sz = (size_t)a.S * 4;
    const int qlen = (a.S + Q - 1) / Q;
    for (int item = w; item < n; item += W) {
        const int e = __builtin_amdgcn_readfirstlane(item / Q), q = item - e * Q;
        const int kap = g * a.Kg + list[e];
        const size_t slot = (size_t)rho * a.K + kap;
        pk_ci32* ch = (pk_ci32*)(a.child_all + slot * 2);
        const cdbl* P = (const cdbl*)(a.Pmat_all + slot * 32);
        const int c0 = ch[0], c1 = ch[1];
        double Pl[16], Pr[16];
#pragma unroll
        for (int j = 0; j < 16; ++j) { Pl[j] = P[j]; Pr[j] = P[16 + j]; }
        const double* Lp = c0 < a.N ? a.leaves + (size_t)c0 * node_sz : a.pool + (size_t)(c0 - a.N) * node_sz;
        const double* Rp = c1 < a.N ? a.leaves + (size_t)c1 * node_sz : a.pool + (size_t)(c1 - a.N) * node_sz;
        double* out = a.pool + slot * node_sz;
        const int s0 = q * qlen, s1 = s0 + qlen < a.S ? s0 + qlen : a.S;
        for (int s = s0 + lane; s < s1; s += U * 64) {
            double Lv[U][4], Rv[U][4];
#pragma unroll
            for (int u = 0; u < U; ++u) {
                const int su = s + u * 64 < s1 ? s + u * 64 : s;
                pk_load4(Lp + (size_t)su * 4, Lv[u]);
                pk_load4(Rp + (size_t)su * 4, Rv[u]);
            }
#pragma unroll
            for (int u = 0; u < U; ++u) {
                double o[4];
                pk_merge_site(Lv[u], Rv[u], Pl, Pr, o);
                if (s + u * 64 < s1) pk_store4(out + (size_t)(s + u * 64) * 4, o);
            }
        }
        if (lane == 0) a.mark[(size_t)rho * a.K + kap] = 1u;
    }
}

template <int LP>
__global__ __launch_bounds__(64, LP == 64 ? 5 : 1) void pk_rank_book_chain(const pk_rank_args a, int item_wgs) {
    extern __shared__ __attribute__((aligned(16))) char smem[];
    if ((int)blockIdx.x < item_wgs) {
        pk_mat_listed(a, (int)blockIdx.x, (int)threadIdx.x);
        return;
    }
    const int lane = threadIdx.x, sub = lane / LP, sl = lane & (LP - 1);
    const int count = a.tab_ptrs ? a.Kloc : a.K;
    int idx = ((int)blockIdx.x - item_wgs) * (64 / LP) + sub;
    if (idx >= count) idx = count - 1;
    const int kg = a.tab_ptrs ? a.k0 + idx : idx;
    const pk_book_lds L = pk_book_carve(smem + (size_t)sub * pk_book_lds_bytes(a.N), a.N);
    const bool local = kg >= a.k0 && kg < a.k0 + a.Kloc;
    pk_book_packed<LP, LP == 64, true>(a, kg, local, L, sl, lane);
    pk_book_tail<LP>(a, kg, local, false, a.mirror && a.r > 0, L, sl, lane);
}

__device__ __forceinline__ void pk_build_leaf_table(const double* __restrict__ P , double (*tab)[4], int t) {
    if (t < 16) tab[t >> 2][t & 3] = P[t];
    else if (t < 20) {
        const int j = t - 16;
        tab[4][j] = pm_fma(1.0, P[12 + j], pm_fma(1.0, P[8 + j], pm_fma(1.0, P[4 + j], 1.0 * P[j])));
    }
}

__device__ __forceinline__ void pk_merge_epilogue(const pk_rank_args& a, int k, int kg, double tot) {
    const double* ax = a.aux + (size_t)k * PK_AUX;
    const double fl = ax[AUX_SUM_REM] + tot;
    const double ll = ((fl + ax[AUX_FPRIOR]) + ax[AUX_LPRIOR]) + ax[AUX_RPRIOR];
    const double lw = (((ll - ax[AUX_LL_TILDE]) - ax[AUX_PAREN]) + ax[AUX_LOGV]) - ax[AUX_Q];
    a.nodell[a.N + a.r * a.K + kg] = tot;
    a.rootll_new[(size_t)kg * a.N + (a.n - 2)] = tot;
    a.ll_r[kg] = ll;
    a.logw_r[kg] = lw;
}

__global__ __launch_bounds__(256) void pk_tile_epilogue(const pk_rank_args a) {
    const int k = blockIdx.x * blockDim.x + threadIdx.x;
    if (k >= a.Kloc) return;
    const double* tv = a.tilev + (size_t)k * a.ntiles;
    double tot = tv[0];
    for (int t = 1; t < a.ntiles; ++t) tot = tot + tv[t];
    pk_merge_epilogue(a, k, a.k0 + k, tot);
}

__global__ void pk_fix_rootll(double* __restrict__ rootll_new, const double* __restrict__ nodell_row, int K, int N, int n,
                              int k0, int Kloc) {
    const int kg = blockIdx.x * blockDim.x + threadIdx.x;
// ... 532 lines not shown
        ro = *(pk_gu32c*)(roff + (u + 192u) * 4u);
        pk_pat_entry<CL, CR>(B, (cw >> 8) & 0xffu, u + 64u, (unsigned int)U, Pl, Pr, tabL, tabR, pi, ulik, flag);
        lo >>= 16;
    }
    if (nU & 1) pk_pat_entry<CL, CR>(A, (unsigned int)lo & 0xffu, u, (unsigned int)U, Pl, Pr, tabL, tabR, pi, ulik, flag);
    if (threadIdx.x == 0) ulik[U] = 1.0;
}
__device__ __forceinline__ void pk_pat_request(pk_u4& n0, pk_u4& n1, const char* pimg, int Jc) {
    const unsigned int o = (unsigned int)Jc * (2u * PK_PAT_HALF_BYTES) + (threadIdx.x & 63u) * 16u;
    n0 = *(pk_gu4c*)(pimg + o);
    n1 = *(pk_gu4c*)(pimg + o + (unsigned int)PK_PAT_HALF_BYTES);
}
__device__ __forceinline__ void pk_pat_walk(int s1, const char* pimg, pk_u4 n0, pk_u4 n1, const double* ulik, pm_lp& col, pm_lp_flag& flag) {
    const char* ub = (const char*)ulik;
    int n = __builtin_amdgcn_readfirstlane((s1 + 63) >> 6), Jc = 0;
    #pragma unroll 1
    for (;;) {
        const unsigned int w[8] = {n0.x, n0.y, n0.z, n0.w, n1.x, n1.y, n1.z, n1.w};
        if (n > 16) pk_pat_request(n0, n1, pimg, Jc + 1);
#pragma unroll
        for (int j = 0; j < 16; j += 2) {
            if (n < j + 2) {
                if (n == j + 1) pm_lp_mul_normal(col, *(const double*)(ub + (w[j >> 1] & 0xffffu)));
                break;
            }
            const double xa = *(const double*)(ub + (w[j >> 1] & 0xffffu));
            const double xb = *(const double*)(ub + (w[j >> 1] >> 16));
            pm_lp_mul2_spec_q(col, xa, xb, flag);
        }
        if (n <= 16) break;
        n -= 16; ++Jc;
    }
}
struct pk_pat_args { const char* pimg; const char* roff; long long rep_delta ; int U; };
typedef __attribute__((address_space(4))) const pk_pat_args pk_pat_kargs;
template <bool CL, bool CR>
__device__ __forceinline__ bool pk_rows_pat(int s1, const char* bl, const char* br, const char* rl, pk_pat_kargs* pa, const double (&Pl)[16],
                                            const double (&Pr)[16], const double (*tabL)[4], const double (*tabR)[4],
                                            const double (&pi)[4], double* ulik, pm_lp& col) {
    pm_lp_flag flag = pm_lp_flag_init();
    const char* pimg = pa->pimg;
    pk_u4 n0, n1;
    if constexpr (CL || CR) pk_pat_request(n0, n1, pimg, 0);
    pk_pat_phase1<CL, CR>(pa->U, bl, br, rl, pa->roff, Pl, Pr, tabL, tabR, pi, ulik, flag);
    if constexpr (!(CL || CR)) pk_pat_request(n0, n1, pimg, 0);
    pk_wave_lds_fence();
    pk_pat_walk(s1, pimg, n0, n1, ulik, col, flag);
    return pm_lp_flag_set(flag);
}
template <bool CL, bool CR>
__device__ __forceinline__ pm_lp pk_rows_general_v(int s0, int s1, const char* bl, const char* br, const pk_cdbl* Pc, const pk_cdbl* pik,
                                                   double (*tabL)[4], double (*tabR)[4], double* lik25) {
    const double pi[4] = {pik[0], pik[1], pik[2], pik[3]};
    double Pl[16], Pr[16];
#pragma unroll
    for (int u = 0; u < 16; ++u) {
        Pl[u] = CL ? 0.0 : Pc[u];
        Pr[u] = CR ? 0.0 : Pc[16 + u];
    }
    pk_rowregs A;
    pm_lp col = pm_lp_init();
    if constexpr (CL || CR) {
        pk_cstream c;
        pk_cs_request<CL, CR>(c, bl, br, s0 >> 10);
        pk_rows_load_u<CL, CR>(A, bl, br, s0 + (int)(threadIdx.x & 63), s1);
        pk_rows_run_packed<CL, CR>(s0, s1, bl, br, A, c, Pl, Pr, tabL, tabR, lik25, pi, col);
    } else {
        pk_rows_load<CL, CR>(A, bl, br, s0 + (int)(threadIdx.x & 63), s1);
        pk_rows_run<CL, CR>(s0, s1, bl, br, A, Pl, Pr, tabL, tabR, lik25, pi, col);
    }
    return col;
}
__device__ __forceinline__ pm_lp pk_rows_general(unsigned int fl, int s0, int s1, const char* bl, const char* br, const double* Pu,
                                                 const double* pi4, double (*tabL)[4], double (*tabR)[4], double* lik25) {
    fl = (unsigned int)__builtin_amdgcn_readfirstlane((int)fl);
    s0 = __builtin_amdgcn_readfirstlane(s0);
    s1 = __builtin_amdgcn_readfirstlane(s1);
    bl = pk_uniform_ptr(bl);
    br = pk_uniform_ptr(br);
    const pk_cdbl* Pc = (const pk_cdbl*)pk_uniform_ptr(Pu);
    const pk_cdbl* pik = (const pk_cdbl*)pk_uniform_ptr(pi4);
    if ((fl & 3u) == 3u) return pk_rows_general_v<true, true>(s0, s1, bl, br, Pc, pik, tabL, tabR, lik25);
    if (fl & 1u) return pk_rows_general_v<true, false>(s0, s1, bl, br, Pc, pik, tabL, tabR, lik25);
    if (fl & 2u) return pk_rows_general_v<false, true>(s0, s1, bl, br, Pc, pik, tabL, tabR, lik25);
    return pk_rows_general_v<false, false>(s0, s1, bl, br, Pc, pik, tabL, tabR, lik25);
}
template <bool CL, bool CR>
__device__ __forceinline__ bool pk_rows_loop_pat(int s1, const char* bl, const char* br, const double* Pu, const pk_cdbl* Pc,
                                                 double (*tabL)[4], double (*tabR)[4], const pk_cdbl* pik, pm_lp& col, pk_pat_kargs* pa,
                                                 double* ulik) {
    static_assert(!(CL && CR), "an uncoded side");
    const double pi[4] = {pik[0], pik[1], pik[2], pik[3]};
    double Pl[16], Pr[16];
#pragma unroll
    for (int u = 0; u < 16; ++u) {
        Pl[u] = CL ? 0.0 : Pc[u];
        Pr[u] = CR ? 0.0 : Pc[16 + u];
    }
    const char* rl = nullptr;
    if constexpr (CL != CR) {
#pragma unroll
        for (int u = 0; u < 16; ++u) asm volatile("" : "+s"(CL ? Pr[u] : Pl[u]));
        rl = (CL ? bl : br) + pa->rep_delta;
        if constexpr (CL) pk_build_leaf_table(Pu, tabL, (int)(threadIdx.x & 63));
        else pk_build_leaf_table(Pu + 16, tabR, (int)(threadIdx.x & 63));
        pk_wave_lds_fence();
    }
    return __any(pk_rows_pat<CL, CR>(s1, bl, br, rl, pa, Pl, Pr, tabL, tabR, pi, ulik, col));
}
template <bool CL, bool CR>
__device__ __forceinline__ bool pk_rows_loop_rec(int s0, int s1, const char* bl, const char* br, const double* Pu, const pk_cdbl* Pc,
                                                 double (*tabL)[4], double (*tabR)[4], double* lik25, const pk_cdbl* pik, pm_lp& col,
                                                 pk_pat_kargs* pa, double* ulik) {
    if constexpr (!(CL && CR)) {
        if (pa->U != 0) return pk_rows_loop_pat<CL, CR>(s1, bl, br, Pu, Pc, tabL, tabR, pik, col, pa, ulik);
    }
    const int lane = threadIdx.x & 63;
    const double pi[4] = {pik[0], pik[1], pik[2], pik[3]};
    double Pl[16], Pr[16];
#pragma unroll
    for (int u = 0; u < 16; ++u) {
        Pl[u] = CL ? 0.0 : Pc[u];
        Pr[u] = CR ? 0.0 : Pc[16 + u];
    }
    if constexpr (CL != CR) {
#pragma unroll
        for (int u = 0; u < 16; ++u) asm volatile("" : "+s"(CL ? Pr[u] : Pl[u]));
    }
    pk_rowregs A;
    pk_cstream c;
    if constexpr (CL || CR) {
        pk_cs_request<CL, CR>(c, bl, br, s0 >> 10);
        pk_rows_load_u<CL, CR>(A, bl, br, s0 + lane, s1);
    } else {
        pk_rows_load<CL, CR>(A, bl, br, s0 + lane, s1);
    }
    bool redo = (s0 & 1023) != 0;
    if constexpr (CL && CR) {
        const bool special = pk_build_lik25_direct(Pu, pi, lik25, lane);
        if (lane == PK_PAD_CODE * 6) lik25[PK_PAD_CODE * 6] = 1.0;
        pk_wave_lds_fence();
        redo = redo || __any(special);
    } else if constexpr (CL) {
        pk_build_leaf_table(Pu, tabL, lane);
        pk_wave_lds_fence();
    } else if constexpr (CR) {
        pk_build_leaf_table(Pu + 16, tabR, lane);
        pk_wave_lds_fence();
    }
    if constexpr (CL || CR) {
        if (!redo) {
            bool flag;
            if constexpr (CL && CR) flag = pk_rows_fast_cc(s0, s1, bl, br, c, lik25, col);
            else flag = pk_rows_fast_mixed<CL, CR>(s0, s1, bl, br, A, c, Pl, Pr, tabL, tabR, pi, col);
            redo = __any(flag);
        }
        return redo;
    } else {
        pk_rows_run<CL, CR>(s0, s1, bl, br, A, Pl, Pr, tabL, tabR, lik25, pi, col);
        return false;
    }
}
struct pk_merge_kernarg { const unsigned long long* rec; const double* Pmat; int S, T, ntiles; double* tilev; pk_pi4 pi4; pk_pat_args pat; };
__global__ __launch_bounds__(64) __attribute__((amdgpu_waves_per_eu(7, 8), amdgpu_num_vgpr(32)))
void pk_rank_merge_nostore(const unsigned long long* __restrict__ rec, const double* __restrict__ Pmat, int S, int T, int ntiles,
                           double* __restrict__ tilev, const pk_pi4 pi4, const pk_pat_args pat) {
    __shared__ __attribute__((aligned(16))) double tabL[PK_PAD_CODE + 1][4], tabR[PK_PAD_CODE + 1][4];
    __shared__ double lik25[PK_PAD_CODE * 6 + 1];
    extern __shared__ __attribute__((aligned(16))) double pk_ulik[];
    const int item = (int)blockIdx.x;
    const int k = __builtin_amdgcn_readfirstlane(ntiles == 1 ? item : item / ntiles), tau = item - k * ntiles;
    const int s0 = __builtin_amdgcn_readfirstlane(tau * T), s1 = __builtin_amdgcn_readfirstlane(s0 + T < S ? s0 + T : S);
    const pk_cu64* rc = (const pk_cu64*)(rec + (size_t)k * PK_REC);
    const double* Pu = Pmat + (size_t)k * 32;
    const pk_cdbl* Pc = (const pk_cdbl*)Pu;
    PK_TOUCH4_DECL;
    PK_TOUCH4_256(Pu);
    unsigned int fl = (unsigned int)rc[REC_FLAGS];
    const char* bl = pk_uniform_ptr((const void*)rc[REC_BASE_L]);
    const char* br = pk_uniform_ptr((const void*)rc[REC_BASE_R]);
    PK_TOUCH4_END(fl);
    static_assert(offsetof(pk_merge_kernarg, pi4) == 40 && offsetof(pk_merge_kernarg, pat) == 72 && sizeof(pk_merge_kernarg) == 104,
                  "the kernel's argument segment");
    pk_pat_kargs* pa = (pk_pat_kargs*)((__attribute__((address_space(4))) const char*)__builtin_amdgcn_kernarg_segment_ptr() +
                                       offsetof(pk_merge_kernarg, pat));
    const pk_cdbl* pi = (const pk_cdbl*)((__attribute__((address_space(4))) const char*)__builtin_amdgcn_kernarg_segment_ptr() +
                                         offsetof(pk_merge_kernarg, pi4));
    pm_lp col = pm_lp_init();
    bool redo;
    if (fl & 1u) {
        if (fl & 2u) redo = pk_rows_loop_rec<true, true>(s0, s1, bl, br, Pu, Pc, tabL, tabR, lik25, pi, col, pa, pk_ulik);
        else redo = pk_rows_loop_rec<true, false>(s0, s1, bl, br, Pu, Pc, tabL, tabR, lik25, pi, col, pa, pk_ulik);
    } else {
        if (fl & 2u) redo = pk_rows_loop_rec<false, true>(s0, s1, bl, br, Pu, Pc, tabL, tabR, lik25, pi, col, pa, pk_ulik);
        else redo = pk_rows_loop_rec<false, false>(s0, s1, bl, br, Pu, Pc, tabL, tabR, lik25, pi, col, pa, pk_ulik);
    }
    if (redo) col = pk_rows_general(fl, s0, s1, bl, br, Pu, (const double*)pi, tabL, tabR, lik25);
    const double tot = pk_wave_tree_sum(pm_lp_finish(col));
    if (threadIdx.x == 0) {
        if (ntiles != 1) {
            tilev[(size_t)k * ntiles + tau] = tot;
        } else {
            const pk_cdbl* ax = (const pk_cdbl*)rc;
            const double fl2 = ax[AUX_SUM_REM] + tot;
            const double ll = ((fl2 + ax[AUX_FPRIOR]) + ax[AUX_LPRIOR]) + ax[AUX_RPRIOR];
            const double lw = (((ll - ax[AUX_LL_TILDE]) - ax[AUX_PAREN]) + ax[AUX_LOGV]) - ax[AUX_Q];
            *(pk_gd*)rc[REC_NODELL] = tot;
            *(pk_gd*)rc[REC_ROOTLL] = tot;
            *(pk_gd*)rc[REC_LL] = ll;
            *(pk_gd*)rc[REC_LOGW] = lw;
        }
    }
}

#define PK_MAX_SITE_TILE 4096
#define PK_STORE_STAGE_BYTES 8192
template <bool CL, bool CR, bool STORE>
__device__ __forceinline__ void pk_store_tile(int s0, int s1, int wv, int lane, const double* Lp, const double* Rp, const uint8_t* Lc,
                                              const uint8_t* Rc, double* out, const double (&Pl)[16], const double (&Pr)[16],
                                              const double (*tabL)[4], const double (*tabR)[4], const double (&pi)[4], double* likbuf,
                                              double* stage ) {
    const char* bl = pk_uniform_ptr(CL ? (const void*)Lc : (const void*)Lp);
    const char* br = pk_uniform_ptr(CR ? (const void*)Rc : (const void*)Rp);
    char* ob = const_cast<char*>(pk_uniform_ptr(out));
    pk_rowregs A, B;
    int u = s0 + 64 * wv;
    if (u >= s1) return;
    pk_rows_load<CL, CR>(A, bl, br, u + lane, s1);
// ... 579 lines not shown
```

phylo_amd/csrc/phylo_site_patterns.h:

```cpp
#pragma once
#include <stddef.h>
#include <stdint.h>
#include <string.h>

#include <vector>

#include "phylo_packed_codes.h"

#define PK_PAT_MAX_U 512
#define PK_PAT_REP_WORDS 1024
#define PK_PAT_HALF_BYTES 1024
#define PK_PAT_IMAGE_MAX_U 8191

enum { PK_PAT_OFF = 0, PK_PAT_AUTO = 1, PK_PAT_FORCE = 2 };

static inline size_t pk_pat_image_bytes(int S) { return (size_t)pk_packed_chunks(S) * 2 * PK_PAT_HALF_BYTES; }
static inline size_t pk_pat_rep_bytes() { return (size_t)PK_PAT_REP_WORDS * 4; }
static inline size_t pk_pat_offset(int N, int S) { return (pk_codes_image_bytes(N, S) + 15) & ~(size_t)15; }
static inline size_t pk_pat_rep_offset(int N, int S) { return pk_pat_offset(N, S) + pk_pat_image_bytes(S); }
static inline size_t pk_pat_leaf_offset(int N, int S) { return pk_pat_rep_offset(N, S) + pk_pat_rep_bytes(); }
static inline size_t pk_leaf_image_bytes(int N, int S) { return pk_pat_leaf_offset(N, S) + pk_packed_bytes(N, S); }
static inline size_t pk_pat_lds_bytes(int U) { return ((size_t)((U + 63) / 64) * 64 + 1) * 8; }

static inline int pk_pat_columns(const uint8_t* codes, int N, int S, int32_t* pat, int32_t* rep) {
// ... 21 lines not shown
            if (eq) { u = cand; break; }
        }
        if (u < 0) {
            u = U++;
            rep[u] = s;
            slot[i] = u;
        }
        pat[s] = u;
    }
    return U;
}
static inline void pk_pat_pack_image(const int32_t* pat, int S, int U, uint16_t* image) {
    const size_t n = pk_pat_image_bytes(S) / 2;
    const uint16_t pad = (uint16_t)(8 * U);
    for (size_t i = 0; i < n; ++i) image[i] = pad;
    const int nsteps = (S + 63) / 64;
    for (int q = 0; q < nsteps; ++q) {
        const int cnt = S - 64 * q < 64 ? S - 64 * q : 64;
        uint16_t* d = image + ((size_t)(q / PK_CHUNK_STEPS) * 2 + (q % PK_CHUNK_STEPS) / 8) * (PK_PAT_HALF_BYTES / 2) + q % 8;
        const int32_t* p = pat + (size_t)64 * q;
        for (int c = 0; c < cnt; ++c) d[c * 8] = (uint16_t)(8 * p[c]);
    }
}
static inline void pk_pat_rep_offsets(const int32_t* rep, int U, uint32_t* off) {
    for (int u = 0; u < PK_PAT_REP_WORDS; ++u) off[u] = u < U ? 32u * (uint32_t)rep[u] : 0u;
}
static inline void pk_pat_rep_leaf_image(const uint8_t* codes, int N, int S, const int32_t* rep, int U, uint8_t* packed, size_t stride) {
    std::vector<uint8_t> cu((size_t)U);
    for (int leaf = 0; leaf < N; ++leaf) {
        for (int u = 0; u < U; ++u) cu[u] = codes[(size_t)leaf * S + rep[u]];
        pk_pack_leaf_codes(cu.data(), 1, U, packed + (size_t)leaf * stride);
    }
}
static inline int pk_pat_build(const uint8_t* codes, int N, int S, uint8_t* tables) {
    std::vector<int32_t> pat((size_t)S), rep((size_t)S);
    const int U = pk_pat_columns(codes, N, S, pat.data(), rep.data());
    if (U <= PK_PAT_MAX_U) {
        pk_pat_pack_image(pat.data(), S, U, (uint16_t*)tables);
        pk_pat_rep_offsets(rep.data(), U, (uint32_t*)(tables + pk_pat_image_bytes(S)));
        pk_pat_rep_leaf_image(codes, N, S, rep.data(), U, tables + pk_pat_image_bytes(S) + pk_pat_rep_bytes(), pk_packed_leaf_bytes(S));
    }
    return U;
}

#define PK_PAT_C_STEP 38
#define PK_PAT_C_PHASE1 33
#define PK_PAT_C_WALK 7
#define PK_PAT_C_FIXED 30
static inline bool pk_pat_valid(int S, int U, bool coded, int ntiles) {
    return coded && ntiles == 1 && S >= 1 && U >= 1 && U <= PK_PAT_MAX_U;
}
static inline bool pk_pat_take(int S, int U, bool coded, int ntiles, int sw) {
    if (sw == PK_PAT_OFF || !pk_pat_valid(S, U, coded, ntiles)) return false;
    if (sw == PK_PAT_FORCE) return true;
    const long nS = (S + 63) / 64, nU = (U + 63) / 64;
    return 10 * (nU * PK_PAT_C_PHASE1 + nS * PK_PAT_C_WALK + PK_PAT_C_FIXED) <= 8 * nS * PK_PAT_C_STEP;
}
```

phylo_amd/csrc/phylo_sweep_plan.h:

```cpp
#pragma once

#include <cstddef>
#include <cstdint>
#include <cstdio>

struct sweep_limits {
    int max_groups;
    int twist_max_m, twist_max_j;
    int mat_group;
    int scan_fold_max_kg;
    int scan_lds512_max_kg;
    int kept_bits_taxa;
    int one_tile_max_s;
    int small_max_kg, small_max_kloc;
    int book_packed8_min;
    int sorted_min_draws;
};

struct sweep_facts {
    int N, K, Kloc, S, G, M, world;
    int ntiles;
    bool transport;
    bool device_exchange;
    bool jc;
    bool coded_leaves;
    bool twisting, keep_graph, eager_nodes, time_kernels;
    bool env_eager_nodes, env_rehearse_sharded, env_replicated_book;
};

struct sweep_plan {
    int R, G, Kg;
    bool twist, graph, timek;
    bool one_tile;
    bool lazy;
    bool shard_form;
    bool replicated_book;
    bool local_book;
    bool book_mat;
    bool mat_by_draws;
    bool want_rdraw;
    bool use_rec;
    bool sorted_prologue;
    bool mat_grouped;
    bool mat_draws_grouped;
    int book_width;
    bool step_a_work;
    bool mat_after_book;
    bool mat_barrier;
    bool twist_ll;
    bool twist_tables;
    bool tile_epilogue;
    bool fix_rootll;
    bool fold_logz;
    int lse_stride;
    bool no_store_last;
    bool final_missing;
    bool last_graph_eager;
    int gather_launches;
};

inline bool sweep_eager_nodes(bool flag, bool env) { return flag || env; }

inline int sweep_book_width(int N, int nbook, const sweep_limits& L) {
    if (N <= 16) return nbook >= L.book_packed8_min ? 8 : 16;
    return N <= 32 ? 32 : 64;
}

inline bool sweep_refuses_batch(const sweep_facts& f, const sweep_limits& L, char* msg, size_t n) {
    const bool sharded = f.world != 1;
    if (f.G < 1 || f.G > L.max_groups || f.K % f.G != 0)
        return snprintf(msg, n, "a batch needs 1 <= G <= %d sweeps and K = %d divisible by G (got %d)", L.max_groups, f.K, f.G), true;
    if (f.G > 1 && f.twisting) return snprintf(msg, n, "batched sweeps need the plain proposal (PHYLO_TWISTING is set)"), true;
    if (f.G > 1 && f.keep_graph) {
        if (sharded || f.transport) return snprintf(msg, n, "batched sweeps with PHYLO_KEEP_GRAPH need an unsharded context"), true;
        if (f.S > L.one_tile_max_s)
            return snprintf(msg, n, "batched sweeps with PHYLO_KEEP_GRAPH need S <= 4096 sites (got %d)", f.S), true;
    }
    return false;
}
inline bool sweep_refuses_form(const sweep_facts& f, const sweep_limits& L, char* msg, size_t n) {
    const bool sharded = f.world != 1;
    if (f.twisting) {
        if (f.M < 1 || f.M > L.twist_max_m)
            return snprintf(msg, n, "twisting needs 1 <= M <= %d (got %d)", L.twist_max_m, f.M), true;
        const size_t Jmax = (size_t)(f.N * (f.N - 1) / 2) * (size_t)f.M;
        if (Jmax > (size_t)L.twist_max_j) return snprintf(msg, n, "twisting: C(N,2)*M = %zu exceeds %d", Jmax, L.twist_max_j), true;
    }
    if (f.keep_graph && sharded) {
        if (f.twisting) return snprintf(msg, n, "PHYLO_KEEP_GRAPH with PHYLO_TWISTING needs an unsharded context"), true;
        if (f.S > L.one_tile_max_s)
            return snprintf(msg, n, "PHYLO_KEEP_GRAPH on a sharded context needs S <= 4096 sites (got %d)", f.S), true;
// ... 4 lines not shown
inline sweep_plan sweep_plan_form(const sweep_facts& f, const sweep_limits& L) {
    sweep_plan p{};
    const int N = f.N, K = f.K, Kl = f.Kloc, S = f.S;
    p.R = N - 1; p.G = f.G; p.Kg = K / f.G;
    p.twist = f.twisting; p.graph = f.keep_graph; p.timek = f.time_kernels;
    const bool eager = sweep_eager_nodes(f.eager_nodes, f.env_eager_nodes);
    const bool one_tile = p.one_tile = S <= L.one_tile_max_s;
    p.lazy = !p.twist && (!p.graph || one_tile) && !eager;
    p.shard_form = f.world > 1 || (f.transport && f.env_rehearse_sharded);
    p.replicated_book = f.env_replicated_book || (p.graph && f.world > 1);
    p.local_book = !p.twist && p.shard_form && !p.replicated_book;
    p.book_mat = p.lazy && f.world == 1 && !f.transport && N <= 64 && one_tile && f.G == 1 && Kl <= L.small_max_kloc;
    const bool mat_small = p.Kg <= L.small_max_kg && Kl <= L.small_max_kloc;
    p.mat_by_draws = p.lazy && p.local_book && one_tile && (mat_small || (p.Kg % L.mat_group == 0 && Kl % L.mat_group == 0));
    p.mat_draws_grouped = !mat_small;
    p.want_rdraw = p.book_mat || p.mat_by_draws;
    p.no_store_last = !p.graph && !eager;
    p.final_missing = p.no_store_last && !p.lazy;
    p.use_rec = !p.twist && Kl == K && p.lazy;
    p.sorted_prologue = !p.twist && !f.jc && 2L * p.R * Kl >= L.sorted_min_draws;
    p.mat_grouped = one_tile && Kl > L.small_max_kloc;
    p.step_a_work = p.lazy && p.local_book;
    p.mat_after_book = p.lazy && !p.local_book && !p.book_mat;
    p.mat_barrier = f.transport;
    p.book_width = p.twist ? 0 : sweep_book_width(N, p.local_book ? Kl : K, L);
    p.twist_ll = p.twist && f.coded_leaves;
    p.twist_tables = p.twist && f.transport;
    p.tile_epilogue = f.ntiles > 1;
    p.fix_rootll = f.transport && !p.local_book;
    p.fold_logz = p.Kg <= L.scan_fold_max_kg;
    p.lse_stride = f.G > 1 ? p.R + 1 : 0;
    p.last_graph_eager = p.graph && !p.lazy && !p.twist && one_tile && f.world == 1 && Kl == K && N > L.kept_bits_taxa;
    p.gather_launches = (p.graph && f.world > 1) ? (f.device_exchange ? 4 : 2) : 0;
    return p;
}

enum sweep_scan_form {
    SCAN_MULTI = 0,
    SCAN_LDS_512 = 1,
    SCAN_LDS_1024 = 2,
    SCAN_IN_PLACE = 3
};
inline sweep_scan_form sweep_scan_form_of(int Kg, int multi_min, bool wanted, const sweep_limits& L) {
    if (Kg > multi_min && wanted) return SCAN_MULTI;
    if (Kg <= L.scan_lds512_max_kg) return SCAN_LDS_512;
    if (Kg <= L.scan_fold_max_kg) return SCAN_LDS_1024;
    return SCAN_IN_PLACE;
}

struct sweep_chain_form {
    bool taken;
    int item_waves;
    int parts;
};
inline sweep_chain_form sweep_chain_form_of(const sweep_plan& p, int S, int multi_min, int scan_ancestors, const sweep_limits& L) {
    const sweep_chain_form no{};
    if (scan_ancestors == 0) return no;
    if (!(p.use_rec && p.mat_after_book)) return no;
    if (p.mat_barrier) return no;
    if (p.R < 2) return no;
    const sweep_scan_form s = sweep_scan_form_of(p.Kg, multi_min, true, L);
    if (s != SCAN_LDS_512 && s != SCAN_LDS_1024) return no;
    sweep_chain_form f{};
    f.taken = true;
    f.parts = (S + 127) / 128 < 8 ? (S + 127) / 128 : 8;
    f.item_waves = p.Kg * f.parts < 128 ? p.Kg * f.parts : 128;
// ... 43 lines not shown
inline bool persist_refuses_shape(const persist_facts& f, const persist_limits& L) {
    if (!f.one_launch) return true;
    if (f.world != 1 || f.transport) return true;
    if (f.twisting || f.keep_graph || f.time_kernels) return true;
    if (sweep_eager_nodes(f.eager_nodes, f.env_eager_nodes)) return true;
    if (f.N > L.max_taxa || f.N < 2) return true;
    if (f.K / f.G > L.max_kg) return true;
    if (f.S > L.max_s) return true;
    return false;
}

inline persist_grid persist_plan_of(const persist_facts& f, const persist_limits& L) {
    const persist_grid no{};
    if (persist_refuses_shape(f, L)) return no;
    if (f.blocks_per_cu < 1 || f.n_cus < 1) return no;
    const int Kg = f.K / f.G;
    int Wt = f.persist_wgs > 0 ? f.persist_wgs : f.n_cus;
    if (Wt > f.n_cus * f.blocks_per_cu) Wt = f.n_cus * f.blocks_per_cu;
    if (Wt < f.G) return no;
    int Wg = Wt / f.G;
    if (Wg > Kg) Wg = Kg;
    while (Wg > 1 && Kg % Wg) --Wg;
    const int m = Kg / Wg;
    if (m > L.max_m) return no;
    const size_t lds = L.lds_bytes(f.N, m, Kg);
    if (lds > L.max_lds) return no;
    return persist_grid{true, Wg, m, f.persist_nt, lds};
}

inline uint32_t sweep_plan_mask(const sweep_plan& p) {
    const bool b[] = {p.twist, p.graph, p.timek, p.lazy, p.shard_form, p.replicated_book, p.local_book, p.book_mat, p.mat_by_draws,
                      p.want_rdraw, p.use_rec, p.sorted_prologue, p.mat_grouped, p.mat_draws_grouped, p.step_a_work, p.mat_after_book,
                      p.mat_barrier, p.fix_rootll, p.fold_logz, p.no_store_last, p.final_missing, p.last_graph_eager,
                      p.one_tile, p.twist_ll, p.twist_tables, p.tile_epilogue, p.lse_stride != 0};
    static_assert(sizeof b / sizeof b[0] <= 28, "bits 28..31 hold book_width / 8");
    uint32_t m = (uint32_t)(p.book_width / 8) << 28;
    for (size_t i = 0; i < sizeof b / sizeof b[0]; ++i) m |= b[i] ? 1u << i : 0u;
    return m;
}
```

Measured before the change: 709.5 billion particle-site-likelihoods/s.

## Precompute per-clade site-pattern tables to compress likelihood work per subtree

Adds host-built tables for every leaf subset (clade bitmask) of up to 12 taxa. Each table records the distinct site patterns restricted to that clade and maps every site to its class. The bookkeeping kernels track clade bitmasks per particle, so the merge/likelihood kernels can evaluate only the unique columns for each subtree instead of all global patterns. This trades a tables upload of up to 32 MB and extra bitmask state and LDS per particle for fewer partial-likelihood evaluations at internal nodes.

```diff
diff --git a/include/phylo_hip.h b/include/phylo_hip.h
--- a/include/phylo_hip.h
+++ b/include/phylo_hip.h
@@ -154,6 +154,9 @@
                               uint8_t* rep_leaf, int64_t rep_leaf_cap);
 int phylo_debug_site_patterns_rule(int S, int U, int coded, int ntiles, int sw);
 int phylo_debug_site_patterns_of(phylo_ctx* ctx, int32_t* U, int32_t* taken);
+int phylo_debug_clade_patterns_rule(int pat_taken, int N, int S, int U, int sw, int64_t* bytes);
+int phylo_debug_clade_tables(const uint8_t* codes, int N, int S, int32_t* U, int64_t* layout, uint8_t* tables, int64_t cap, uint16_t* cls);
+int phylo_debug_clade_patterns_of(phylo_ctx* ctx, int32_t* eligible, int32_t* taken, int64_t* bytes);
 int phylo_debug_reverse_plan_batch(int N, int K, int G, int S, uint32_t switches, int64_t n_slow, int TS, int64_t coeff_wgs,
                                    int passes_in_flight, uint32_t* mask);
 int phylo_debug_tree_plan(int N, int K, int G, int world, int64_t n_clades, int64_t n_topologies, int kept_whole, int force_wide,
diff --git a/phylo_amd/_ffi.py b/phylo_amd/_ffi.py
--- a/phylo_amd/_ffi.py
+++ b/phylo_amd/_ffi.py
@@ -25,7 +25,7 @@
     "phylo_sweep_async", "phylo_sweep_batch_async", "phylo_sweep_batch_begin", "phylo_sweep_fetch_logz", "phylo_sweep_begin", "phylo_sweep_step", "phylo_sweep_step_a", "phylo_sweep_step_group", "phylo_sweep_finish", "phylo_sweep_fetch",
     "phylo_synchronize", "phylo_sweep_node", "phylo_sweep_backward", "phylo_sweep_backward_batch",
     "phylo_tree_summary", "phylo_tree_summary_fetch", "phylo_tree_branches", "phylo_tree_branches_fetch",
-    "phylo_math_probe", "phylo_debug_frechet", "phylo_debug_stamps", "phylo_debug_reverse_lists", "phylo_debug_lookahead_lists", "phylo_debug_reverse_plan", "phylo_debug_reverse_plan_batch", "phylo_debug_sweep_plan", "phylo_debug_sweep_chain", "phylo_debug_sweep_chain_of", "phylo_debug_scan_ancestors", "phylo_debug_pack_leaf_codes", "phylo_debug_site_patterns", "phylo_debug_site_patterns_rule", "phylo_debug_site_patterns_of", "phylo_debug_tree_plan", "phylo_debug_tree_branches_of", "phylo_debug_scan_form", "phylo_debug_persist_plan", "phylo_debug_persist_of", "phylo_debug_device_lists", "phylo_debug_device_lists_of", "phylo_debug_remote_cache", "phylo_debug_site_product",
+    "phylo_math_probe", "phylo_debug_frechet", "phylo_debug_stamps", "phylo_debug_reverse_lists", "phylo_debug_lookahead_lists", "phylo_debug_reverse_plan", "phylo_debug_reverse_plan_batch", "phylo_debug_sweep_plan", "phylo_debug_sweep_chain", "phylo_debug_sweep_chain_of", "phylo_debug_scan_ancestors", "phylo_debug_pack_leaf_codes", "phylo_debug_site_patterns", "phylo_debug_site_patterns_rule", "phylo_debug_site_patterns_of", "phylo_debug_clade_patterns_rule", "phylo_debug_clade_tables", "phylo_debug_clade_patterns_of", "phylo_debug_tree_plan", "phylo_debug_tree_branches_of", "phylo_debug_scan_form", "phylo_debug_persist_plan", "phylo_debug_persist_of", "phylo_debug_device_lists", "phylo_debug_device_lists_of", "phylo_debug_remote_cache", "phylo_debug_site_product",
     "phylo_vi_gradients", "phylo_vi_gradients_batch", "phylo_vi_apply",
     "phylo_site_tile", "phylo_set_site_tile", "phylo_get_site_tile",
     "phylo_comm_unique_id", "phylo_comm_init", "phylo_comm_share", "phylo_comm_allgather", "phylo_comm_max", "phylo_comm_barrier",
@@ -217,6 +217,62 @@
     if rc < 0:
         raise PhyloError(rc, lib.phylo_last_error(None).decode())
     return bool(rc)
+
+
+CLADE_MAX_TAXA = 12
+CLADE_MAX_BYTES = 32 << 20
+
+
+def debug_clade_patterns_rule(N, S, U, pat_taken=True, switch=None):
+    lib = load()
+    nbytes = C.c_int64(0)
+    rc = lib.phylo_debug_clade_patterns_rule(C.c_int(int(pat_taken)), C.c_int(N), C.c_int(S), C.c_int(U), C.c_int(SITE_PATTERN_SWITCH[switch]),
+                                             C.byref(nbytes))
+    if rc < 0:
+        raise PhyloError(rc, lib.phylo_last_error(None).decode())
+    return bool(rc), nbytes.value
+
+
+def debug_clade_tables(codes):
+    lib = load()
+    cd = np.ascontiguousarray(codes, dtype=np.uint8)
+    if cd.ndim != 2:
+        raise ValueError("codes must be [N][S]")
+    N, S = cd.shape
+    U = C.c_int32(0)
+    lay = (C.c_int64 * 5)()
+    rc = lib.phylo_debug_clade_tables(_ptr(cd), C.c_int(N), C.c_int(S), C.byref(U), lay, None, C.c_int64(0), None)
+    if rc:
+        raise PhyloError(rc, lib.phylo_last_error(None).decode())
+    codes_bytes, rep_bytes, image_bytes, stride, total = (int(x) for x in lay)
+    buf = np.full(total, 0xff, dtype=np.uint8)
+    cls = np.full((1 << N) * U.value, 0xffff, dtype=np.uint16)
+    rc = lib.phylo_debug_clade_tables(_ptr(cd), C.c_int(N), C.c_int(S), C.byref(U), lay, _ptr(buf), C.c_int64(total), _ptr(cls))
+    if rc:
+        raise PhyloError(rc, lib.phylo_last_error(None).decode())
+    blocks = {}
+    for Z in range(1 << N):
+        if bin(Z).count("1") < 3:
+            continue
+        b = buf[codes_bytes + Z * stride: codes_bytes + (Z + 1) * stride]
+        blocks[Z] = {"U": int(b[:4].view(np.uint32)[0]), "rep_off": b[256:256 + rep_bytes].view(np.uint32).copy(),
+                     "image": b[256 + rep_bytes:].view(np.uint16).reshape(-1, 2, 64, 8).copy()}
+    return {"U": U.value, "codes": buf[:codes_bytes].reshape(N, -1).copy(), "cls": cls.reshape(1 << N, U.value), "blocks": blocks,
+            "layout": {"codes_bytes": codes_bytes, "rep_bytes": rep_bytes, "image_bytes": image_bytes, "stride": stride, "total": total}}
+
+
+def debug_sweep_plan_clade(N, K, S, clade_tables=True, **kw):
+    lib = load()
+    sw = sum(1 << SWEEP_PLAN_SWITCHES.index(name) for name in kw.get("switches", ())) | (64 if clade_tables else 0)
+    mask = C.c_uint32(0)
+    launches = (C.c_int32 * (max(N, 1) + 1))()
+    K_local = kw.get("K_local")
+    rc = lib.phylo_debug_sweep_plan(C.c_int(N), C.c_int(K), C.c_int(K if K_local is None else K_local), C.c_int(S), C.c_int(kw.get("G", 1)),
+                                    C.c_int(kw.get("M", 1)), C.c_int(kw.get("world", 1)), C.c_int(int(kw.get("transport", False))),
+                                    C.c_uint32(kw.get("flags", 0)), C.c_uint32(sw), C.byref(mask), launches)
+    if rc:
+        raise PhyloError(rc, lib.phylo_last_error(None).decode())
+    return bool(mask.value >> 27 & 1)
 
 
 TREE_SUMMARY_BUFS = ("u", "U", "bits", "kA", "kB", "val", "scan", "weight", "srt", "hp", "o_cbits", "o_cw", "o_tw", "child", "slot", "o_cg",
@@ -931,6 +987,11 @@
         self._check(self._lib.phylo_debug_site_patterns_of(self._h, C.byref(U), C.byref(taken)))
         return U.value, bool(taken.value)
 
+    def debug_clade_patterns(self):
+        el, taken, nbytes = C.c_int32(0), C.c_int32(0), C.c_int64(0)
+        self._check(self._lib.phylo_debug_clade_patterns_of(self._h, C.byref(el), C.byref(taken), C.byref(nbytes)))
+        return bool(el.value), bool(taken.value), nbytes.value
+
     def debug_tree_branches(self):
         wide, cbits, tbits = C.c_int32(0), C.c_int32(0), C.c_int32(0)
         self._check(self._lib.phylo_debug_tree_branches_of(self._h, C.byref(wide), C.byref(cbits), C.byref(tbits)))
diff --git a/phylo_amd/csrc/phylo_hip.hip b/phylo_amd/csrc/phylo_hip.hip
--- a/phylo_amd/csrc/phylo_hip.hip
+++ b/phylo_amd/csrc/phylo_hip.hip
@@ -70,6 +70,7 @@
     int scan_multi_min = 4096;
     int scan_ancestors = 1;
     int site_patterns = PK_PAT_AUTO;
+    int clade_patterns = PK_CLADE_AUTO;
     int trees_chunk = 0;
     int rell_chunk = 0;
     void read() {
@@ -88,6 +89,7 @@
         { const char* e = getenv("PHYLO_TREE_WIDE_KEYS"); tree_wide_keys = e && atoi(e) != 0; }
         { const char* e = getenv("PHYLO_REMOTE_CACHE_CAP"); remote_cache_cap = e ? atoi(e) : 0; }
         { const char* e = getenv("PHYLO_SITE_PATTERNS"); site_patterns = !e ? PK_PAT_AUTO : !strcmp(e, "force") ? PK_PAT_FORCE : atoi(e) == 0 ? PK_PAT_OFF : PK_PAT_AUTO; }
+        { const char* e = getenv("PHYLO_CLADE_PATTERNS"); clade_patterns = !e ? PK_CLADE_AUTO : !strcmp(e, "force") ? PK_CLADE_FORCE : atoi(e) == 0 ? PK_CLADE_OFF : PK_CLADE_AUTO; }
         { const char* e = getenv("PHYLO_SCAN_MULTI_MIN"); scan_multi_min = e ? atoi(e) : 4096; }
         { const char* e = getenv("PHYLO_SCAN_ANCESTORS"); scan_ancestors = e ? atoi(e) : 1; }
         { const char* e = getenv("PHYLO_TREES_CHUNK"); trees_chunk = e ? atoi(e) : 0; }
@@ -134,6 +136,13 @@
     uint8_t* d_pat = nullptr;
     int pat_U = 0;
     bool leaves_coded = false;
+    uint8_t* d_clade = nullptr;
+    uint8_t* h_clade_p = nullptr;
+    size_t clade_cap = 0;
+    pk_clade_layout clade_layout{};
+    bool clade_ready = false;
+    hipEvent_t ev_clade = nullptr;
+    int32_t* d_bits[2] = {nullptr, nullptr};
     uint32_t* d_pair_hist = nullptr;
     bool hist_ready = false, codes_valid = false;
     double* d_pool = nullptr;
@@ -401,6 +410,8 @@
     c->pctr_dirty = false;
     if (c->d_tilev) (void)hipFree(c->d_tilev);
     c->d_tilev = nullptr;
+    if (c->d_bits[0]) (void)hipFree(c->d_bits[0]);
+    c->d_bits[0] = c->d_bits[1] = nullptr;
     void* ptrs[] = {c->d_pool, c->d_nodell, c->d_bl, c->d_br, c->d_Pmat, c->d_logw, c->d_ll, c->d_aux, c->d_lse, c->d_group_seeds,
                     c->d_tables, (void*)c->d_tab_ptrs, c->d_child, c->d_merges, c->d_anc,
                     c->d_cdf[0], c->d_cdf[1], c->d_anc_next, c->d_adopt_list, c->d_adopt_cnt, c->d_counter, (void*)c->d_pool_ptrs, c->d_mark, c->d_sync, c->d_mirror, c->d_cache, c->d_rec};
@@ -784,7 +795,7 @@
     if (c->bgstream) (void)hipStreamSynchronize(c->bgstream);
     phylo_comm_destroy(&c->comm);
     free_sweep_state(c);
-    void* ptrs[] = {c->d_Q, c->d_ldf, c->d_leaves, c->d_leaf_codes};
+    void* ptrs[] = {c->d_Q, c->d_ldf, c->d_leaves, c->d_leaf_codes, c->d_clade};
     for (void* p : ptrs)
         if (p) (void)hipFree(p);
     for (auto& b : c->scratch)
@@ -827,6 +838,8 @@
     if (c->h_model_p) (void)hipHostFree(c->h_model_p);
     if (c->ev_leaves) (void)hipEventDestroy(c->ev_leaves);
     if (c->h_leaves_p) (void)hipHostFree(c->h_leaves_p);
+    if (c->ev_clade) (void)hipEventDestroy(c->ev_clade);
+    if (c->h_clade_p) (void)hipHostFree(c->h_clade_p);
     if (c->stream) (void)hipStreamDestroy(c->stream);
     delete c;
     return PHYLO_OK;
@@ -892,11 +905,31 @@
         c->leaves_coded = ok && !c->env.no_leaf_codes;
         c->hist_ready = false;
         c->pat_U = 0;
+        c->clade_ready = false;
         if (ok) {
             pk_pack_leaf_codes(codes, c->N, c->S, codes + pk_packed_offset(c->N, c->S));
-            c->pat_U = pk_pat_build(codes, c->N, c->S, codes + pk_pat_offset(c->N, c->S));
+            std::vector<int32_t> pat, rep;
+            c->pat_U = pk_pat_build(codes, c->N, c->S, codes + pk_pat_offset(c->N, c->S), pat, rep);
             const size_t up_bytes = c->pat_U <= PK_PAT_MAX_U ? code_bytes : pk_codes_image_bytes(c->N, c->S);
             HIPCHK(c, hipMemcpyAsync(c->d_leaf_codes, codes, up_bytes, hipMemcpyHostToDevice, c->stream));
+            if (pk_clade_take(pk_pat_take(c->S, c->pat_U, c->leaves_coded, 1, c->env.site_patterns), c->N, c->S, c->pat_U, c->env.clade_patterns)) {
+                const pk_clade_layout L = pk_clade_layout_of(c->N, c->S, c->pat_U);
+                if (L.total > c->clade_cap) {
+                    if (c->d_clade) HIPCHK(c, hipFree(c->d_clade));
+                    if (c->h_clade_p) HIPCHK(c, hipHostFree(c->h_clade_p));
+                    c->d_clade = nullptr; c->h_clade_p = nullptr; c->clade_cap = 0;
+                    HIPCHK(c, hipMalloc((void**)&c->d_clade, L.total));
+                    HIPCHK(c, hipHostMalloc((void**)&c->h_clade_p, L.total));
+                    c->clade_cap = L.total;
+                }
+                if (!c->ev_clade) HIPCHK(c, hipEventCreateWithFlags(&c->ev_clade, hipEventDisableTiming));
+                else HIPCHK(c, hipEventSynchronize(c->ev_clade));
+                pk_clade_build(codes, c->N, c->S, pat.data(), rep.data(), c->pat_U, c->h_clade_p, nullptr);
+                HIPCHK(c, hipMemcpyAsync(c->d_clade, c->h_clade_p, L.total, hipMemcpyHostToDevice, c->stream));
+                HIPCHK(c, hipEventRecord(c->ev_clade, c->stream));
+                c->clade_layout = L;
+                c->clade_ready = true;
+            }
         }
     }
     if (pinned) HIPCHK(c, hipEventRecord(c->ev_leaves, c->stream));
@@ -2142,6 +2175,7 @@
     sweep_facts_flags(f, flags);
     f.env_eager_nodes = c->env.eager_nodes; f.env_rehearse_sharded = c->env.rehearse_sharded;
     f.env_replicated_book = c->env.replicated_book;
+    f.clade_tables = c->clade_ready && pk_pat_take(c->S, c->pat_U, c->leaves_coded, c->ntiles, c->env.site_patterns);
     return f;
 }
 
@@ -2250,6 +2284,10 @@
         if (p.twist) CHK(sweep_alloc_twist_history(c, M));
     }
     if (p.want_rdraw && !c->d_rdraw) CHK(dalloc(c, &c->d_rdraw, (size_t)p.R * c->K));
+    if (p.clade_pat && !c->d_bits[0]) {
+        CHK(dalloc(c, &c->d_bits[0], 2 * (size_t)c->K * c->N));
+        c->d_bits[1] = c->d_bits[0] + (size_t)c->K * c->N;
+    }
     return PHYLO_OK;
 }
 
@@ -2267,6 +2305,7 @@
         pa.group_seeds = G > 1 ? (const uint64_t*)c->d_group_seeds : (const uint64_t*)nullptr;
         pa.rdraw = p.want_rdraw ? c->d_rdraw : (unsigned long long*)nullptr;
         pa.roots = t_roots; pa.cnt = t_cnt; pa.rootll = t_rootll; pa.nodell = c->d_nodell; pa.K = K; pa.N = N;
+        pa.bits = p.clade_pat ? c->d_bits[0] : (int32_t*)nullptr;
         pa.mark = p.lazy ? c->d_mark : (unsigned int*)nullptr;
         pa.mark_words = p.lazy ? (unsigned int)mark_words : 0u;
         const int NT = p.sorted_prologue ? 256 : 64;
@@ -2467,6 +2506,7 @@
         b.roots_old = c->d_roots[cur]; b.cnt_old = c->d_cnt[cur];
         b.roots_new = c->d_roots[nxt]; b.cnt_new = c->d_cnt[nxt];
         b.rootll_old = c->d_rootll[cur]; b.rootll_new = c->d_rootll[nxt];
+        if (p.clade_pat) { b.bits_old = c->d_bits[cur]; b.bits_new = c->d_bits[nxt]; }
     }
     if (p.local_book) {
         b.tab_ptrs = c->d_tab_ptrs;
@@ -2584,11 +2624,16 @@
 static int step_book(phylo_ctx* c, const pk_rank_args& b) {
     const sweep_plan& p = c->run.plan;
     const int K = c->K, w = p.book_width;
-    const size_t lds = pk_book_lds_bytes(c->N);
+    const size_t lds = pk_book_lds_bytes(c->N) + (p.clade_pat ? pk_book_bits_lds_bytes(c->N) : 0);
     if (p.book_mat && b.r > 0) {
         const int lp = w < 16 ? 16 : w, per = PK_COLS / lp;
         const int bb = cdiv(K, per);
         const dim3 grid(bb + K);
+        if (p.clade_pat) {
+            if (lp != 16) return fail(c, PHYLO_ESTATE, "step_book: clade patterns at %d lanes", lp);
+            hipLaunchKernelGGL(pk_rank_book_mat_clade<16>, grid, dim3(PK_COLS), lds * per, c->stream, b, bb);
+            return launch_check(c, "pk_rank_book_mat");
+        }
         switch (lp) {
         case 16: hipLaunchKernelGGL(pk_rank_book_mat<16>, grid, dim3(PK_COLS), lds * per, c->stream, b, bb); break;
         case 32: hipLaunchKernelGGL(pk_rank_book_mat<32>, grid, dim3(PK_COLS), lds * per, c->stream, b, bb); break;
@@ -2602,6 +2647,12 @@
     if (ch.taken) {
         const int items = b.r > 0 ? p.G * ch.item_waves : 0;
         const dim3 grid(items + cdiv(K, per));
+        if (p.clade_pat) {
+            if (w == 8) hipLaunchKernelGGL(pk_rank_book_chain_clade<8>, grid, dim3(64), lds * per, c->stream, b, items);
+            else if (w == 16) hipLaunchKernelGGL(pk_rank_book_chain_clade<16>, grid, dim3(64), lds * per, c->stream, b, items);
+            else return fail(c, PHYLO_ESTATE, "step_book: clade patterns at %d lanes", w);
+            return launch_check(c, "pk_rank_book_chain");
+        }
         switch (w) {
         case 8: hipLaunchKernelGGL(pk_rank_book_chain<8>, grid, dim3(64), lds * per, c->stream, b, items); break;
         case 16: hipLaunchKernelGGL(pk_rank_book_chain<16>, grid, dim3(64), lds * per, c->stream, b, items); break;
@@ -2612,6 +2663,12 @@
         return launch_check(c, "pk_rank_book_chain");
     }
     const dim3 grid(cdiv(p.local_book ? c->Kloc : K, per));
+    if (p.clade_pat) {
+        if (w == 8) hipLaunchKernelGGL(pk_rank_book_packed_clade<8>, grid, dim3(64), lds * per, c->stream, b);
+        else if (w == 16) hipLaunchKernelGGL(pk_rank_book_packed_clade<16>, grid, dim3(64), lds * per, c->stream, b);
+        else return fail(c, PHYLO_ESTATE, "step_book: clade patterns at %d lanes", w);
+        return launch_check(c, "pk_rank_book_packed");
+    }
     switch (w) {
     case 8: hipLaunchKernelGGL(pk_rank_book_packed<8>, grid, dim3(64), lds * per, c->stream, b); break;
     case 16: hipLaunchKernelGGL(pk_rank_book_packed<16>, grid, dim3(64), lds * per, c->stream, b); break;
@@ -2634,9 +2691,16 @@
     } else if (b.rec) {
         pk_pi4 pi4;
         memcpy(pi4.v, c->h_model_p + 16, sizeof pi4.v);
-        pk_pat_args pat = {nullptr, nullptr, 0, 0};
+        pk_pat_args pat = {nullptr, nullptr, 0, 0, 0u, 0u, nullptr};
         size_t lds = 0;
-        if (pat_on(c)) {
+        if (p.clade_pat) {
+            const pk_clade_layout& L = c->clade_layout;
+            pat.clade = (const char*)c->d_clade + L.codes_bytes;
+            pat.cstride = (unsigned int)L.stride; pat.crep = (unsigned int)L.rep_bytes;
+            pat.rep_delta = (long long)(c->d_clade - c->d_leaf_packed);
+            pat.U = c->pat_U;
+            lds = pk_pat_lds_bytes(c->pat_U);
+        } else if (pat_on(c)) {
             pat.pimg = (const char*)c->d_pat;
             pat.roff = (const char*)c->d_pat + pk_pat_image_bytes(S);
             pat.rep_delta = (long long)((c->d_pat + pk_pat_image_bytes(S) + pk_pat_rep_bytes()) - c->d_leaf_packed);
@@ -3735,7 +3799,7 @@
     f.transport = transport != 0;
     sweep_facts_flags(f, flags);
     f.env_eager_nodes = switches & 1; f.env_rehearse_sharded = switches & 2; f.env_replicated_book = switches & 4;
-    f.jc = switches & 8; f.coded_leaves = switches & 16; f.device_exchange = switches & 32;
+    f.jc = switches & 8; f.coded_leaves = switches & 16; f.device_exchange = switches & 32; f.clade_tables = switches & 64;
     char why[160];
     if (sweep_refuses_batch(f, k_sweep_limits, why, sizeof why) || sweep_refuses_form(f, k_sweep_limits, why, sizeof why))
         return fail(nullptr, PHYLO_EINVAL, "%s", why);
@@ -3834,6 +3898,38 @@
     if (!c->have_leaves) return fail(c, PHYLO_ESTATE, "phylo_debug_site_patterns_of needs leaves");
     *U = c->pat_U;
     *taken = pat_on(c) ? 1 : 0;
+    return PHYLO_OK;
+}
+
+int phylo_debug_clade_patterns_rule(int pat_taken, int N, int S, int U, int sw, int64_t* bytes) {
+    if (N < 1 || S < 1 || U < 0 || sw < PK_CLADE_OFF || sw > PK_CLADE_FORCE) {
+        (void)fail(nullptr, PHYLO_EINVAL, "phylo_debug_clade_patterns_rule: bad arguments");
+        return -1;
+    }
+    if (bytes) *bytes = (int64_t)pk_clade_layout_of(N, S, U).total;
+    return pk_clade_take(pat_taken != 0, N, S, U, sw) ? 1 : 0;
+}
+
+int phylo_debug_clade_tables(const uint8_t* codes, int N, int S, int32_t* U, int64_t* layout, uint8_t* tables, int64_t cap, uint16_t* cls) {
+    if (N < 1 || N > PK_CLADE_MAX_N || S < 1 || !codes || !U || !layout) return fail(nullptr, PHYLO_EINVAL, "phylo_debug_clade_tables: bad arguments");
+    std::vector<int32_t> pat((size_t)S), rp((size_t)S);
+    *U = pk_pat_columns(codes, N, S, pat.data(), rp.data());
+    const pk_clade_layout L = pk_clade_layout_of(N, S, *U);
+    layout[0] = (int64_t)L.codes_bytes; layout[1] = (int64_t)L.rep_bytes; layout[2] = (int64_t)L.image_bytes;
+    layout[3] = (int64_t)L.stride; layout[4] = (int64_t)L.total;
+    if (!tables) return PHYLO_OK;
+    if (*U > PK_PAT_MAX_U) return fail(nullptr, PHYLO_EINVAL, "phylo_debug_clade_tables: U = %d exceeds %d", *U, PK_PAT_MAX_U);
+    if (cap < (int64_t)L.total) return fail(nullptr, PHYLO_EINVAL, "phylo_debug_clade_tables: the tables take %lld bytes (got %lld)", (long long)L.total, (long long)cap);
+    pk_clade_build(codes, N, S, pat.data(), rp.data(), *U, tables, cls);
+    return PHYLO_OK;
+}
+
+int phylo_debug_clade_patterns_of(phylo_ctx* c, int32_t* eligible, int32_t* taken, int64_t* bytes) {
+    if (!c || !eligible || !taken || !bytes) return fail(c, PHYLO_EINVAL, "phylo_debug_clade_patterns_of: NULL argument");
+    if (!c->have_leaves) return fail(c, PHYLO_ESTATE, "phylo_debug_clade_patterns_of needs leaves");
+    *eligible = (c->clade_ready && pat_on(c)) ? 1 : 0;
+    *taken = c->run.plan.clade_pat ? 1 : 0;
+    *bytes = c->clade_ready ? (int64_t)c->clade_layout.total : 0;
     return PHYLO_OK;
 }
 
diff --git a/phylo_amd/csrc/phylo_kernels.h b/phylo_amd/csrc/phylo_kernels.h
--- a/phylo_amd/csrc/phylo_kernels.h
+++ b/phylo_amd/csrc/phylo_kernels.h
@@ -162,6 +162,7 @@
     double* rootll;
     const double* nodell;
     int K, N;
+    int32_t* bits;
     unsigned int* mark;
     unsigned int mark_words;
     int draw_blocks, init_blocks, mark_blocks;
@@ -256,6 +257,7 @@
                 p.roots[i] = i % p.N;
                 p.cnt[i] = 1;
                 p.rootll[i] = p.nodell[i % p.N];
+                if (p.bits) p.bits[i] = 1 << (i % p.N);
             }
         }
     } else if (b < p.draw_blocks + p.init_blocks + p.mark_blocks) {
@@ -583,12 +585,14 @@
     const int32_t* adopt_list;
     const int32_t* adopt_cnt;
     int item_waves, item_parts;
+    const int32_t* bits_old; int32_t* bits_new;
 };
 
 struct pk_book_lds {
     double *ord_ll, *ord_ldf, *hbl, *hbr, *anc_ll, *ldf;
     uint32_t* key; int32_t *ro, *co, *ord_cnt;
     double* aux; int32_t* misc;
+    int32_t* bo;
 };
 __host__ __device__ inline size_t pk_book_lds_bytes(int N) {
     const size_t n4 = ((size_t)N + 3) & ~(size_t)3;
@@ -609,9 +613,17 @@
     L.co = L.ro + n4;
     L.ord_cnt = L.co + n4;
     L.misc = L.ord_cnt + n4;
+    L.bo = nullptr;
     return L;
 }
-
+__host__ __device__ inline size_t pk_book_bits_lds_bytes(int N) { return (((size_t)N + 3) & ~(size_t)3) * 4; }
+__device__ __forceinline__ pk_book_lds pk_book_carve_sub(char* smem, int sub, int groups, int N) {
+    pk_book_lds L = pk_book_carve(smem + (size_t)sub * pk_book_lds_bytes(N), N);
+    L.bo = (int32_t*)(smem + (size_t)groups * pk_book_lds_bytes(N) + (size_t)sub * pk_book_bits_lds_bytes(N));
+    return L;
+}
+
+template <bool BITS = false>
 __device__ __forceinline__ void pk_rec_write(const pk_rank_args& a, int k, int kg, int t, const pk_book_lds& L) {
     const size_t node_sz = (size_t)a.S * 4;
     unsigned long long v;
@@ -632,6 +644,7 @@
         v = (unsigned long long)(a.logw_r + kg);
     } else {
         v = a.leaf_codes ? (unsigned long long)((L.misc[0] < a.N ? 1 : 0) | (L.misc[1] < a.N ? 2 : 0)) : 0ull;
+        if constexpr (BITS) v |= (unsigned long long)(unsigned int)L.misc[2] << 2;
     }
     a.rec[(size_t)k * PK_REC + t] = v;
 }
@@ -672,7 +685,7 @@
     return lo;
 }
 
-template <int LP, bool KEY_LOOP, bool ANC_IN = false>
+template <int LP, bool KEY_LOOP, bool ANC_IN = false, bool BITS = false>
 __device__ __forceinline__ void pk_book_packed(const pk_rank_args& a, int kg, bool local, const pk_book_lds& L, int sl, int lane) {
     const int n = a.n, N = a.N, k = kg - a.k0;
     const int grp = a.group_seeds ? kg / a.Kg : 0;
@@ -723,6 +736,11 @@
         }
         #pragma unroll 1
         for (int i = sl; i < n; i += LP) { L.ro[i] = ro[i]; L.co[i] = co[i]; L.anc_ll[i] = rl[i]; }
+        if constexpr (BITS) {
+            const int32_t* bo = a.bits_old + (size_t)anc * N;
+            #pragma unroll 1
+            for (int i = sl; i < n; i += LP) L.bo[i] = bo[i];
+        }
         if (sl == 0) {
             L.misc[3] = anc;
             if (local) L.aux[AUX_LL_TILDE] = (a.r > 0) ? a.ll_prev[anc] : a.ll_tilde0;
@@ -776,8 +794,14 @@
             L.ord_cnt[rank] = c;
             L.ord_ll[rank] = xll;
             L.ord_ldf[rank] = L.ldf[c < a.ldf_n ? c : a.ldf_n];
+            if constexpr (BITS) a.bits_new[(size_t)kg * N + rank] = L.bo[i];
         }
         if (sl == 0) {
+            if constexpr (BITS) {
+                const int bnew = L.bo[il] | L.bo[ir];
+                a.bits_new[(size_t)kg * N + (n - 2)] = bnew;
+                L.misc[2] = bnew;
+            }
             const int cnew = L.co[il] + L.co[ir];
             rn[n - 2] = N + a.r * a.K + kg;
             cn[n - 2] = cnew;
@@ -872,7 +896,7 @@
     if (lane == 0) __hip_atomic_store(a.mirror + x, slot + 1, __ATOMIC_RELAXED, __HIP_MEMORY_SCOPE_AGENT);
 }
 
-template <int LP>
+template <int LP, bool BITS = false>
 __device__ __forceinline__ void pk_book_tail(const pk_rank_args& a, int kg, bool local, bool mark, bool cache, const pk_book_lds& L,
                                              int sl, int lane) {
     if (local) {
@@ -884,7 +908,7 @@
         }
         if (a.rec) {
 #pragma unroll
-            for (int t = sl; t < PK_REC_SLOTS; t += LP) pk_rec_write(a, k, kg, t, L);
+            for (int t = sl; t < PK_REC_SLOTS; t += LP) pk_rec_write<BITS>(a, k, kg, t, L);
         }
     }
     if (mark && sl == 0) a.mark[(size_t)(a.r - 1) * a.K + L.misc[3]] = 1u;
@@ -901,18 +925,27 @@
     }
 }
 
-template <int LP>
-__global__ __launch_bounds__(64, LP == 64 ? 5 : 1) void pk_rank_book_packed(const pk_rank_args a) {
-    extern __shared__ __attribute__((aligned(16))) char smem[];
+template <int LP, bool BITS>
+__device__ __forceinline__ void pk_rank_book_packed_body(const pk_rank_args& a, char* smem) {
     const int lane = threadIdx.x, sub = lane / LP, sl = lane & (LP - 1);
     const int count = a.tab_ptrs ? a.Kloc : a.K;
     int idx = blockIdx.x * (64 / LP) + sub;
     if (idx >= count) idx = count - 1;
     const int kg = a.tab_ptrs ? a.k0 + idx : idx;
-    const pk_book_lds L = pk_book_carve(smem + (size_t)sub * pk_book_lds_bytes(a.N), a.N);
+    const pk_book_lds L = BITS ? pk_book_carve_sub(smem, sub, 64 / LP, a.N) : pk_book_carve(smem + (size_t)sub * pk_book_lds_bytes(a.N), a.N);
     const bool local = kg >= a.k0 && kg < a.k0 + a.Kloc;
-    pk_book_packed<LP, LP == 64>(a, kg, local, L, sl, lane);
-    pk_book_tail<LP>(a, kg, local, a.lazy && a.r > 0, a.mirror && a.r > 0, L, sl, lane);
+    pk_book_packed<LP, LP == 64, false, BITS>(a, kg, local, L, sl, lane);
+    pk_book_tail<LP, BITS>(a, kg, local, a.lazy && a.r > 0, a.mirror && a.r > 0, L, sl, lane);
+}
+template <int LP>
+__global__ __launch_bounds__(64, LP == 64 ? 5 : 1) void pk_rank_book_packed(const pk_rank_args a) {
+    extern __shared__ __attribute__((aligned(16))) char smem[];
+    pk_rank_book_packed_body<LP, false>(a, smem);
+}
+template <int LP>
+__global__ __launch_bounds__(64, 1) void pk_rank_book_packed_clade(const pk_rank_args a) {
+    extern __shared__ __attribute__((aligned(16))) char smem[];
+    pk_rank_book_packed_body<LP, true>(a, smem);
 }
 
 __global__ __launch_bounds__(64) void pk_all_marks(const pk_rank_args a) {
@@ -1056,9 +1089,8 @@
     else pk_mat_by_thresholds(a, a.k0 + (int)blockIdx.x);
 }
 
-template <int LP>
-__global__ __launch_bounds__(PK_COLS, 5) void pk_rank_book_mat(const pk_rank_args a, int book_blocks) {
-    extern __shared__ __attribute__((aligned(16))) char smem[];
+template <int LP, bool BITS>
+__device__ __forceinline__ void pk_rank_book_mat_body(const pk_rank_args& a, int book_blocks, char* smem) {
     if ((int)blockIdx.x >= book_blocks) {
         pk_mat_by_thresholds(a, (int)blockIdx.x - book_blocks);
         return;
@@ -1067,9 +1099,19 @@
     int idx = blockIdx.x * (PK_COLS / LP) + sub;
     if (idx >= a.K) idx = a.K - 1;
     const int kg = idx;
-    const pk_book_lds L = pk_book_carve(smem + (size_t)sub * pk_book_lds_bytes(a.N), a.N);
-    pk_book_packed<LP, false>(a, kg, true, L, sl, lane);
-    pk_book_tail<LP>(a, kg, true, a.r > 0, false, L, sl, lane);
+    const pk_book_lds L = BITS ? pk_book_carve_sub(smem, sub, PK_COLS / LP, a.N) : pk_book_carve(smem + (size_t)sub * pk_book_lds_bytes(a.N), a.N);
+    pk_book_packed<LP, false, false, BITS>(a, kg, true, L, sl, lane);
+    pk_book_tail<LP, BITS>(a, kg, true, a.r > 0, false, L, sl, lane);
+}
+template <int LP>
+__global__ __launch_bounds__(PK_COLS, 5) void pk_rank_book_mat(const pk_rank_args a, int book_blocks) {
+    extern __shared__ __attribute__((aligned(16))) char smem[];
+    pk_rank_book_mat_body<LP, false>(a, book_blocks, smem);
+}
+template <int LP>
+__global__ __launch_bounds__(PK_COLS, 5) void pk_rank_book_mat_clade(const pk_rank_args a, int book_blocks) {
+    extern __shared__ __attribute__((aligned(16))) char smem[];
+    pk_rank_book_mat_body<LP, true>(a, book_blocks, smem);
 }
 
 __device__ __forceinline__ const double* pk_node_ptr(const pk_rank_args& a, int id) {
@@ -1129,9 +1171,8 @@
     }
 }
 
-template <int LP>
-__global__ __launch_bounds__(64, LP == 64 ? 5 : 1) void pk_rank_book_chain(const pk_rank_args a, int item_wgs) {
-    extern __shared__ __attribute__((aligned(16))) char smem[];
+template <int LP, bool BITS>
+__device__ __forceinline__ void pk_rank_book_chain_body(const pk_rank_args& a, int item_wgs, char* smem) {
     if ((int)blockIdx.x < item_wgs) {
         pk_mat_listed(a, (int)blockIdx.x, (int)threadIdx.x);
         return;
@@ -1141,10 +1182,20 @@
     int idx = ((int)blockIdx.x - item_wgs) * (64 / LP) + sub;
     if (idx >= count) idx = count - 1;
     const int kg = a.tab_ptrs ? a.k0 + idx : idx;
-    const pk_book_lds L = pk_book_carve(smem + (size_t)sub * pk_book_lds_bytes(a.N), a.N);
+    const pk_book_lds L = BITS ? pk_book_carve_sub(smem, sub, 64 / LP, a.N) : pk_book_carve(smem + (size_t)sub * pk_book_lds_bytes(a.N), a.N);
     const bool local = kg >= a.k0 && kg < a.k0 + a.Kloc;
-    pk_book_packed<LP, LP == 64, true>(a, kg, local, L, sl, lane);
-    pk_book_tail<LP>(a, kg, local, false, a.mirror && a.r > 0, L, sl, lane);
+    pk_book_packed<LP, LP == 64, true, BITS>(a, kg, local, L, sl, lane);
+    pk_book_tail<LP, BITS>(a, kg, local, false, a.mirror && a.r > 0, L, sl, lane);
+}
+template <int LP>
+__global__ __launch_bounds__(64, LP == 64 ? 5 : 1) void pk_rank_book_chain(const pk_rank_args a, int item_wgs) {
+    extern __shared__ __attribute__((aligned(16))) char smem[];
+    pk_rank_book_chain_body<LP, false>(a, item_wgs, smem);
+}
+template <int LP>
+__global__ __launch_bounds__(64, 1) void pk_rank_book_chain_clade(const pk_rank_args a, int item_wgs) {
+    extern __shared__ __attribute__((aligned(16))) char smem[];
+    pk_rank_book_chain_body<LP, true>(a, item_wgs, smem);
 }
 
 __device__ __forceinline__ void pk_build_leaf_table(const double* __restrict__ P , double (*tab)[4], int t) {
@@ -1743,18 +1794,71 @@
         n -= 16; ++Jc;
     }
 }
-struct pk_pat_args { const char* pimg; const char* roff; long long rep_delta ; int U; };
+struct pk_pat_args {
+    const char* pimg; const char* roff; long long rep_delta ; int U;
+    unsigned int cstride, crep;
+    const char* clade;
+};
 typedef __attribute__((address_space(4))) const pk_pat_args pk_pat_kargs;
+template <bool CL, bool CR>
+__device__ __forceinline__ void pk_clade_rows(pk_rowregs& x, const char* bl, const char* br, const char* cb, unsigned int off) {
+    pk_pat_rows<CL, CR>(x, bl, br, off);
+    if constexpr (CL) x.cl = *(pk_gu8c*)(cb + (off >> 5));
+    if constexpr (CR) x.cr = *(pk_gu8c*)(cb + (off >> 5));
+}
+template <bool CL, bool CR>
+__device__ __forceinline__ void pk_clade_entry(const pk_rowregs& X, unsigned int u, unsigned int U, const double (&Pl)[16],
+                                               const double (&Pr)[16], const double (*tabL)[4], const double (*tabR)[4],
+                                               const double (&pi)[4], double* ulik, pm_lp_flag& flag) {
+    double x = pk_rows_lik<CL, CR>(X, Pl, Pr, tabL, tabR, nullptr, pi);
+    x = u < U ? x : 1.0;
+    flag.f = pm_min_u32(flag.f, pm_lp_key(x));
+    ulik[u] = x;
+}
+template <bool CL, bool CR>
+__device__ __forceinline__ void pk_clade_phase1(const char* blk, const char* bl, const char* br, const char* cb, const double (&Pl)[16],
+                                                const double (&Pr)[16], const double (*tabL)[4], const double (*tabR)[4],
+                                                const double (&pi)[4], double* ulik, pm_lp_flag& flag) {
+    static_assert(!(CL && CR), "an uncoded side");
+    const char* roff = blk + PK_CLADE_HDR_BYTES;
+    unsigned int u = threadIdx.x & 63u;
+    pk_rowregs A, B;
+    unsigned int ro = *(pk_gu32c*)(roff + u * 4u);
+    const int U = *(__attribute__((address_space(4))) const int*)blk;
+    pk_clade_rows<CL, CR>(A, bl, br, cb, ro);
+    ro = *(pk_gu32c*)(roff + (u + 64u) * 4u);
+    const int nU = (U + 63) >> 6;
+    #pragma unroll 1
+    for (int t = 0; t < (nU >> 1); ++t, u += 128u) {
+        pk_clade_rows<CL, CR>(B, bl, br, cb, ro);
+        ro = *(pk_gu32c*)(roff + (u + 128u) * 4u);
+        pk_clade_entry<CL, CR>(A, u, (unsigned int)U, Pl, Pr, tabL, tabR, pi, ulik, flag);
+        pk_clade_rows<CL, CR>(A, bl, br, cb, ro);
+        ro = *(pk_gu32c*)(roff + (u + 192u) * 4u);
+        pk_clade_entry<CL, CR>(B, u + 64u, (unsigned int)U, Pl, Pr, tabL, tabR, pi, ulik, flag);
+    }
+    if (nU & 1) pk_clade_entry<CL, CR>(A, u, (unsigned int)U, Pl, Pr, tabL, tabR, pi, ulik, flag);
+    if (threadIdx.x == 0) ulik[U] = 1.0;
+}
 template <bool CL, bool CR>
 __device__ __forceinline__ bool pk_rows_pat(int s1, const char* bl, const char* br, const char* rl, pk_pat_kargs* pa, const double (&Pl)[16],
                                             const double (&Pr)[16], const double (*tabL)[4], const double (*tabR)[4],
-                                            const double (&pi)[4], double* ulik, pm_lp& col) {
+                                            const double (&pi)[4], double* ulik, pm_lp& col, unsigned int Z) {
     pm_lp_flag flag = pm_lp_flag_init();
-    const char* pimg = pa->pimg;
+    const char* pimg;
     pk_u4 n0, n1;
-    if constexpr (CL || CR) pk_pat_request(n0, n1, pimg, 0);
-    pk_pat_phase1<CL, CR>(pa->U, bl, br, rl, pa->roff, Pl, Pr, tabL, tabR, pi, ulik, flag);
-    if constexpr (!(CL || CR)) pk_pat_request(n0, n1, pimg, 0);
+    if (pa->clade != nullptr) {
+        const char* blk = pa->clade + (size_t)(Z * pa->cstride);
+        pimg = blk + PK_CLADE_HDR_BYTES + pa->crep;
+        if constexpr (CL || CR) pk_pat_request(n0, n1, pimg, 0);
+        pk_clade_phase1<CL, CR>(blk, bl, br, rl, Pl, Pr, tabL, tabR, pi, ulik, flag);
+        if constexpr (!(CL || CR)) pk_pat_request(n0, n1, pimg, 0);
+    } else {
+        pimg = pa->pimg;
+        if constexpr (CL || CR) pk_pat_request(n0, n1, pimg, 0);
+        pk_pat_phase1<CL, CR>(pa->U, bl, br, rl, pa->roff, Pl, Pr, tabL, tabR, pi, ulik, flag);
+        if constexpr (!(CL || CR)) pk_pat_request(n0, n1, pimg, 0);
+    }
     pk_wave_lds_fence();
     pk_pat_walk(s1, pimg, n0, n1, ulik, col, flag);
     return pm_lp_flag_set(flag);
@@ -1799,7 +1903,7 @@
 template <bool CL, bool CR>
 __device__ __forceinline__ bool pk_rows_loop_pat(int s1, const char* bl, const char* br, const double* Pu, const pk_cdbl* Pc,
                                                  double (*tabL)[4], double (*tabR)[4], const pk_cdbl* pik, pm_lp& col, pk_pat_kargs* pa,
-                                                 double* ulik) {
+                                                 double* ulik, unsigned int Z) {
     static_assert(!(CL && CR), "an uncoded side");
     const double pi[4] = {pik[0], pik[1], pik[2], pik[3]};
     double Pl[16], Pr[16];
@@ -1817,14 +1921,14 @@
         else pk_build_leaf_table(Pu + 16, tabR, (int)(threadIdx.x & 63));
         pk_wave_lds_fence();
     }
-    return __any(pk_rows_pat<CL, CR>(s1, bl, br, rl, pa, Pl, Pr, tabL, tabR, pi, ulik, col));
+    return __any(pk_rows_pat<CL, CR>(s1, bl, br, rl, pa, Pl, Pr, tabL, tabR, pi, ulik, col, Z));
 }
 template <bool CL, bool CR>
 __device__ __forceinline__ bool pk_rows_loop_rec(int s0, int s1, const char* bl, const char* br, const double* Pu, const pk_cdbl* Pc,
                                                  double (*tabL)[4], double (*tabR)[4], double* lik25, const pk_cdbl* pik, pm_lp& col,
-                                                 pk_pat_kargs* pa, double* ulik) {
+                                                 pk_pat_kargs* pa, double* ulik, unsigned int Z) {
     if constexpr (!(CL && CR)) {
-        if (pa->U != 0) return pk_rows_loop_pat<CL, CR>(s1, bl, br, Pu, Pc, tabL, tabR, pik, col, pa, ulik);
+        if (pa->U != 0) return pk_rows_loop_pat<CL, CR>(s1, bl, br, Pu, Pc, tabL, tabR, pik, col, pa, ulik, Z);
     }
     const int lane = threadIdx.x & 63;
     const double pi[4] = {pik[0], pik[1], pik[2], pik[3]};
@@ -1891,7 +1995,7 @@
     const char* bl = pk_uniform_ptr((const void*)rc[REC_BASE_L]);
     const char* br = pk_uniform_ptr((const void*)rc[REC_BASE_R]);
     PK_TOUCH4_END(fl);
-    static_assert(offsetof(pk_merge_kernarg, pi4) == 40 && offsetof(pk_merge_kernarg, pat) == 72 && sizeof(pk_merge_kernarg) == 104,
+    static_assert(offsetof(pk_merge_kernarg, pi4) == 40 && offsetof(pk_merge_kernarg, pat) == 72 && sizeof(pk_merge_kernarg) == 120,
                   "the kernel's argument segment");
     pk_pat_kargs* pa = (pk_pat_kargs*)((__attribute__((address_space(4))) const char*)__builtin_amdgcn_kernarg_segment_ptr() +
                                        offsetof(pk_merge_kernarg, pat));
@@ -1900,11 +2004,11 @@
     pm_lp col = pm_lp_init();
     bool redo;
     if (fl & 1u) {
-        if (fl & 2u) redo = pk_rows_loop_rec<true, true>(s0, s1, bl, br, Pu, Pc, tabL, tabR, lik25, pi, col, pa, pk_ulik);
-        else redo = pk_rows_loop_rec<true, false>(s0, s1, bl, br, Pu, Pc, tabL, tabR, lik25, pi, col, pa, pk_ulik);
+        if (fl & 2u) redo = pk_rows_loop_rec<true, true>(s0, s1, bl, br, Pu, Pc, tabL, tabR, lik25, pi, col, pa, pk_ulik, fl >> 2);
+        else redo = pk_rows_loop_rec<true, false>(s0, s1, bl, br, Pu, Pc, tabL, tabR, lik25, pi, col, pa, pk_ulik, fl >> 2);
     } else {
-        if (fl & 2u) redo = pk_rows_loop_rec<false, true>(s0, s1, bl, br, Pu, Pc, tabL, tabR, lik25, pi, col, pa, pk_ulik);
-        else redo = pk_rows_loop_rec<false, false>(s0, s1, bl, br, Pu, Pc, tabL, tabR, lik25, pi, col, pa, pk_ulik);
+        if (fl & 2u) redo = pk_rows_loop_rec<false, true>(s0, s1, bl, br, Pu, Pc, tabL, tabR, lik25, pi, col, pa, pk_ulik, fl >> 2);
+        else redo = pk_rows_loop_rec<false, false>(s0, s1, bl, br, Pu, Pc, tabL, tabR, lik25, pi, col, pa, pk_ulik, fl >> 2);
     }
     if (redo) col = pk_rows_general(fl, s0, s1, bl, br, Pu, (const double*)pi, tabL, tabR, lik25);
     const double tot = pk_wave_tree_sum(pm_lp_finish(col));
diff --git a/phylo_amd/csrc/phylo_site_patterns.h b/phylo_amd/csrc/phylo_site_patterns.h
--- a/phylo_amd/csrc/phylo_site_patterns.h
+++ b/phylo_amd/csrc/phylo_site_patterns.h
@@ -77,8 +77,8 @@
         pk_pack_leaf_codes(cu.data(), 1, U, packed + (size_t)leaf * stride);
     }
 }
-static inline int pk_pat_build(const uint8_t* codes, int N, int S, uint8_t* tables) {
-    std::vector<int32_t> pat((size_t)S), rep((size_t)S);
+static inline int pk_pat_build(const uint8_t* codes, int N, int S, uint8_t* tables, std::vector<int32_t>& pat, std::vector<int32_t>& rep) {
+    pat.resize((size_t)S); rep.resize((size_t)S);
     const int U = pk_pat_columns(codes, N, S, pat.data(), rep.data());
     if (U <= PK_PAT_MAX_U) {
         pk_pat_pack_image(pat.data(), S, U, (uint16_t*)tables);
@@ -86,6 +86,10 @@
         pk_pat_rep_leaf_image(codes, N, S, rep.data(), U, tables + pk_pat_image_bytes(S) + pk_pat_rep_bytes(), pk_packed_leaf_bytes(S));
     }
     return U;
+}
+static inline int pk_pat_build(const uint8_t* codes, int N, int S, uint8_t* tables) {
+    std::vector<int32_t> pat, rep;
+    return pk_pat_build(codes, N, S, tables, pat, rep);
 }
 
 #define PK_PAT_C_STEP 38
@@ -101,3 +105,82 @@
     const long nS = (S + 63) / 64, nU = (U + 63) / 64;
     return 10 * (nU * PK_PAT_C_PHASE1 + nS * PK_PAT_C_WALK + PK_PAT_C_FIXED) <= 8 * nS * PK_PAT_C_STEP;
 }
+
+#define PK_CLADE_MAX_N 12
+#define PK_CLADE_MAX_BYTES ((size_t)32 << 20)
+#define PK_CLADE_HDR_BYTES 256
+#define PK_CLADE_DEFAULT 1
+
+enum { PK_CLADE_OFF = 0, PK_CLADE_AUTO = 1, PK_CLADE_FORCE = 2 };
+
+struct pk_clade_layout { size_t codes_bytes, rep_bytes, image_bytes, stride, total; };
+static inline pk_clade_layout pk_clade_layout_of(int N, int S, int U) {
+    pk_clade_layout L;
+    L.codes_bytes = pk_packed_bytes(N, S);
+    L.rep_bytes = (size_t)((U + 63) / 64 + 2) * 256;
+    L.image_bytes = pk_pat_image_bytes(S);
+    L.stride = PK_CLADE_HDR_BYTES + L.rep_bytes + L.image_bytes;
+    L.total = L.codes_bytes + (N <= 30 ? ((size_t)1 << N) : ((size_t)1 << 30)) * L.stride;
+    return L;
+}
+static inline bool pk_clade_take(bool pat_taken, int N, int S, int U, int sw) {
+    if (sw == PK_CLADE_OFF || (sw == PK_CLADE_AUTO && !PK_CLADE_DEFAULT)) return false;
+    if (!pat_taken || N < 3 || N > PK_CLADE_MAX_N) return false;
+    return pk_clade_layout_of(N, S, U).total <= PK_CLADE_MAX_BYTES;
+}
+static inline void pk_clade_build(const uint8_t* codes, int N, int S, const int32_t* pat, const int32_t* rep, int U, uint8_t* out,
+                                  uint16_t* cls_out) {
+    const pk_clade_layout L = pk_clade_layout_of(N, S, U);
+    const size_t leaf_bytes = pk_packed_leaf_bytes(S);
+    memset(out, 0, L.codes_bytes);
+    for (int leaf = 0; leaf < N; ++leaf) memcpy(out + (size_t)leaf * leaf_bytes, codes + (size_t)leaf * S, (size_t)S);
+    std::vector<uint8_t> cu((size_t)N * U);
+    for (int leaf = 0; leaf < N; ++leaf)
+        for (int u = 0; u < U; ++u) cu[(size_t)leaf * U + u] = codes[(size_t)leaf * S + rep[u]];
+    const size_t nimg = L.image_bytes / 2;
+    std::vector<uint16_t> pidx(nimg, (uint16_t)U);
+    std::vector<uint16_t> off8((size_t)U + 1);
+    for (int s = 0; s < S; ++s) {
+        const int q = s / 64, c = s % 64;
+        pidx[((size_t)(q / PK_CHUNK_STEPS) * 2 + (q % PK_CHUNK_STEPS) / 8) * (PK_PAT_HALF_BYTES / 2) + (size_t)c * 8 + q % 8] = (uint16_t)pat[s];
+    }
+    const size_t nZ = (size_t)1 << N;
+    std::vector<uint16_t> cls_own;
+    uint16_t* cls = cls_out;
+    if (!cls) { cls_own.resize(nZ * U); cls = cls_own.data(); }
+    for (int u = 0; u < U; ++u) cls[u] = 0;
+    std::vector<int32_t> stamp((size_t)U * 6, 0);
+    std::vector<uint16_t> id((size_t)U * 6);
+    std::vector<uint32_t> first((size_t)U + 1);
+    const size_t rep_words = L.rep_bytes / 4;
+    for (size_t Z = 1; Z < nZ; ++Z) {
+        int h = 0, leaves = 0;
+        for (int b = 0; b < N; ++b)
+            if (Z >> b & 1) { h = b; ++leaves; }
+        const uint16_t* cp = cls + (Z ^ ((size_t)1 << h)) * U;
+        uint16_t* cz = cls + Z * U;
+        const uint8_t* ch = cu.data() + (size_t)h * U;
+        int n = 0;
+        for (int u = 0; u < U; ++u) {
+            const size_t key = (size_t)cp[u] * 6 + ch[u];
+            const unsigned int fresh = stamp[key] != (int32_t)Z, keep = fresh - 1u;
+            stamp[key] = (int32_t)Z;
+            const uint16_t k = (uint16_t)(((unsigned int)n & ~keep) | (id[key] & keep));
+            id[key] = k;
+            first[n] = 32u * (uint32_t)rep[u];
+            n += fresh;
+            cz[u] = k;
+        }
+        if (leaves < 3) continue;
+        uint8_t* blk = out + L.codes_bytes + Z * L.stride;
+        uint32_t* ro = (uint32_t*)(blk + PK_CLADE_HDR_BYTES);
+        memcpy(ro, first.data(), (size_t)n * 4);
+        for (size_t w = (size_t)n; w < rep_words; ++w) ro[w] = 0u;
+        memset(blk, 0, PK_CLADE_HDR_BYTES);
+        *(uint32_t*)blk = (uint32_t)n;
+        uint16_t* img = (uint16_t*)(blk + PK_CLADE_HDR_BYTES + L.rep_bytes);
+        for (int u = 0; u < U; ++u) off8[u] = (uint16_t)(8 * cz[u]);
+        off8[U] = (uint16_t)(8 * n);
+        for (size_t i = 0; i < nimg; ++i) img[i] = off8[pidx[i]];
+    }
+}
diff --git a/phylo_amd/csrc/phylo_sweep_plan.h b/phylo_amd/csrc/phylo_sweep_plan.h
--- a/phylo_amd/csrc/phylo_sweep_plan.h
+++ b/phylo_amd/csrc/phylo_sweep_plan.h
@@ -26,6 +26,7 @@
     bool coded_leaves;
     bool twisting, keep_graph, eager_nodes, time_kernels;
     bool env_eager_nodes, env_rehearse_sharded, env_replicated_book;
+    bool clade_tables;
 };
 
 struct sweep_plan {
@@ -57,6 +58,7 @@
     bool final_missing;
     bool last_graph_eager;
     int gather_launches;
+    bool clade_pat;
 };
 
 inline bool sweep_eager_nodes(bool flag, bool env) { return flag || env; }
@@ -127,6 +129,7 @@
     p.lse_stride = f.G > 1 ? p.R + 1 : 0;
     p.last_graph_eager = p.graph && !p.lazy && !p.twist && one_tile && f.world == 1 && Kl == K && N > L.kept_bits_taxa;
     p.gather_launches = (p.graph && f.world > 1) ? (f.device_exchange ? 4 : 2) : 0;
+    p.clade_pat = f.clade_tables && p.use_rec && !p.graph && f.ntiles == 1;
     return p;
 }
 
@@ -236,7 +239,7 @@
     const bool b[] = {p.twist, p.graph, p.timek, p.lazy, p.shard_form, p.replicated_book, p.local_book, p.book_mat, p.mat_by_draws,
                       p.want_rdraw, p.use_rec, p.sorted_prologue, p.mat_grouped, p.mat_draws_grouped, p.step_a_work, p.mat_after_book,
                       p.mat_barrier, p.fix_rootll, p.fold_logz, p.no_store_last, p.final_missing, p.last_graph_eager,
-                      p.one_tile, p.twist_ll, p.twist_tables, p.tile_epilogue, p.lse_stride != 0};
+                      p.one_tile, p.twist_ll, p.twist_tables, p.tile_epilogue, p.lse_stride != 0, p.clade_pat};
     static_assert(sizeof b / sizeof b[0] <= 28, "bits 28..31 hold book_width / 8");
     uint32_t m = (uint32_t)(p.book_width / 8) << 28;
     for (size_t i = 0; i < sizeof b / sizeof b[0]; ++i) m |= b[i] ? 1u << i : 0u;
```

Measured after the change: 729.8 billion particle-site-likelihoods/s, median of 6. +2.9%, better.
